# maple3142/gf2bv

Hardware: AMD Instinct MI355X
Metric: GF(2) row-XORs/s (solve_one, dense NxN) (higher is better)
Workload: dtype u64

## Files before the change

### gf2bv_amd/csrc/gf2_kernels.hip.h

```cpp
#pragma once
#include <hip/hip_runtime.h>
#include <stdint.h>
#include <type_traits>

typedef unsigned long long u64;
typedef long long i64;

#define GF2_GMAX 4
#define GF2_TW 2
#define GF2_TW_LOG 1
#define GF2_LPR 1
#define GF2_OWN_LOG 3
#define GF2_FEW_UNITS 8
#ifndef GF2_BATCH
#define GF2_BATCH 4
#endif
#ifndef GF2_UROWS
#define GF2_UROWS 2
#endif

__device__ __forceinline__ long long tidx(long long row, long long word, long long srows)
{
	return ((word >> GF2_TW_LOG) * srows + row) * GF2_TW + (word & (GF2_TW - 1));
}
// ... 2536 lines not shown
			u32x4 v[NB][RB];
			loadm(0, 0); loadm(1, 1);
#pragma unroll
			for (int pre = 0; pre < NB - 1; pre++) issue(v[pre], m0[0], m1[0], pre);
#pragma unroll
			for (int j = 0; j < SEG; j++) {
#pragma unroll
				for (int rr = 0; rr < NR; rr++) {
					const int g = j * NR + rr;
					const int gi = g + NB - 1, ji = gi / NR, ri = gi % NR, ci = ji & 1;
					issue(v[gi % NB], m0[ci], m1[ci], ri);
					if (ri == NR - 1) loadm(ji + 2, ci);
					fold(d[j], v[g % NB]);
				}
			}
		}
#pragma unroll
		for (int j = 0; j < SEG; j++)
			if ((alive >> j) & 1) (Mrow + j * (NW * 64))[ulane] = d[j];
	}
}

#define GF2_U16K_PARAMS u64 *__restrict__ M, i64 rows, i64 srows, int nblk, const int *__restrict__ gprow, const u64 *__restrict__ mult, i64 set_words, \
	int set0, int nsets, const int *__restrict__ blk_first, const int *__restrict__ died, int j_end, int tile_begin, int ntiles, SysStride ss, int chunk_major
#define GF2_U16K_ARGS M, rows, srows, nblk, gprow, mult, set_words, set0, nsets, blk_first, died, j_end, tile_begin, ntiles, ss, chunk_major
template <int SEG, int NT_ = 512, int RB = 8, int NB = 2>
__global__ void __launch_bounds__(NT_)
k_update16k(GF2_U16K_PARAMS)
{
	update16k_body<SEG, NT_, RB, NB>(GF2_U16K_ARGS);
}
#define GF2_WSEG 12
#define GF2_U16K_WIDE(NAME, SEG, RB, NB, VB) \
	__global__ void __launch_bounds__(1024) __attribute__((amdgpu_num_vgpr(VB))) NAME(GF2_U16K_PARAMS) { update16k_body<SEG, 1024, RB, NB>(GF2_U16K_ARGS); }
GF2_U16K_WIDE(k_update16k_wide, GF2_WSEG, 2, 2, 60)

__global__ void __launch_bounds__(512)
k_outer_apply(u64 *__restrict__ M, i64 rows, i64 srows, int nblk, const int *__restrict__ lists, const u64 *__restrict__ Tm, int tile_begin, SysStride ss)
{
	{
		const i64 ao = blockIdx.y * ss.arena_bytes;
		M += blockIdx.y * ss.m_words;
		lists = sys_at(lists, ao); Tm = sys_at(Tm, ao);
	}
	constexpr int NT = 512, NW = 8, SEG = GF2_KMAX * GF2_GMAX * 64 / NT, NQ = GF2_KMAX * GF2_GMAX * 64;
	__shared__ __attribute__((aligned(256))) uint4 tab[2 * 256 * 16];
	__shared__ uint4 stage[GF2_GMAX * 64];
	__shared__ int srcrow[NQ];
	if ((unsigned)(size_t)tab != 0u) __builtin_trap();
	const int lane = threadIdx.x & 63, wv = threadIdx.x >> 6;
	const int wvu = __builtin_amdgcn_readfirstlane(wv);
	for (int t = threadIdx.x; t < NQ; t += NT) srcrow[t] = lists[NQ + GF2_KMAX + t];
	__syncthreads();
	unsigned KC[6];
	{
		const int rq_lo = lane & 7, rq_hi = (lane >> 3) & 1;
#pragma unroll
		for (int v = 0; v < 6; v++) {
			unsigned k = 1u << 24;
#pragma unroll
			for (int b = 0; b < 3; b++) {
				const int s = 3 * v + b;
				if (s < 16) k |= (unsigned)(16 * (8 * ((s >> 3) ^ rq_hi) + (((s & 7) + rq_lo) & 7))) << (8 * b);
			}
			asm volatile("" : "+v"(k));
			KC[v] = k;
		}
	}
	const i64 R64 = (rows + 63) & ~(i64)63;
	uint4 *Mw = reinterpret_cast<uint4 *>(M) + ((i64)tile_begin + blockIdx.x) * srows;
	uint4 d[SEG];
#pragma unroll
	for (int j = 0; j < SEG; j++) d[j] = make_uint4(0, 0, 0, 0);
	uint4 staged = make_uint4(0, 0, 0, 0);
	if (threadIdx.x < GF2_GMAX * 64) { const int sr = srcrow[threadIdx.x]; staged = sr >= 0 ? Mw[sr] : make_uint4(0, 0, 0, 0); }
	const uint4 *tbase = reinterpret_cast<const uint4 *>(Tm);
#pragma unroll 1
	for (int k = 0; k < nblk; k++) {
		const uint4 *mq = tbase + (i64)k * (NQ * 2);
		uint4 A0[SEG], A1[SEG];
#pragma unroll
		for (int j = 0; j < SEG; j++) {
			const int i = (j * NW + wv) * 64 + lane;
			if (((j * NW + wvu) >> 2) < k) { A0[j] = make_uint4(0, 0, 0, 0); A1[j] = A0[j]; }
			else { A0[j] = mq[i * 2]; A1[j] = mq[i * 2 + 1]; }
		}
		__syncthreads();
		if (threadIdx.x < GF2_GMAX * 64) stage[threadIdx.x] = staged;
		__syncthreads();
		for (int e = threadIdx.x; e < 2 * 31 * 16; e += NT) {
			const int sub = e & 15, q = (e >> 4) % 31, grp = (e >> 4) / 31;
			const int idx = q <= 15 ? q : (q - 15) << 4;
			const uint4 *st = stage + (2 * grp + (sub >> 3)) * 64 + 8 * (sub & 7);
			uint4 acc = make_uint4(0, 0, 0, 0);
			int bits = idx;
			while (bits) { const int l = __ffs(bits) - 1; bits &= bits - 1; acc = xor4(acc, st[l]); }
			tab[grp * 4096 + idx * 16 + sub] = acc;
		}
		__syncthreads();
		for (int e = threadIdx.x; e < 2 * 225 * 16; e += NT) {
			const int sub = e & 15, q = (e >> 4) % 225, grp = (e >> 4) / 225;
			const int lo = 1 + q % 15, hi = (1 + q / 15) << 4;
			uint4 *tb = tab + grp * 4096 + sub;
			tb[(lo | hi) * 16] = xor4(tb[lo * 16], tb[hi * 16]);
		}
		if (k + 1 < nblk && threadIdx.x < GF2_GMAX * 64) {
			const int sr = srcrow[(k + 1) * 256 + threadIdx.x];
			staged = sr >= 0 ? Mw[sr] : make_uint4(0, 0, 0, 0);
		}
		__syncthreads();
#pragma unroll
		for (int j = 0; j < SEG; j++) {
			if (((j * NW + wvu) >> 2) < k) continue;
			const uint4 a0 = A0[j], a1 = A1[j];
			const unsigned mw[8] = { a0.x, a0.y, a0.z, a0.w, a1.x, a1.y, a1.z, a1.w };
#pragma unroll
			for (int r = 0; r < 4; r++) {
				const int grp = r >> 1, hf = r & 1;
				u32x4 v[8];
#pragma unroll
				for (int q = 0; q < 8; q++) {
					const int s = 8 * hf + q;
					const unsigned sel = (unsigned)(s % 3) | ((4u + (unsigned)(q & 3)) << 8) | ((grp ? 3u : 12u) << 16) | (12u << 24);
					const unsigned at = __builtin_amdgcn_perm(mw[2 * (2 * grp + hf) + (q >> 2)], KC[s / 3], sel);
					v[q] = *(lds_u4_ptr)(size_t)at;
				}
#pragma unroll
				for (int h = 0; h < 4; h++) {
					d[j].x = __builtin_amdgcn_bitop3_b32(d[j].x, v[2 * h].x, v[2 * h + 1].x, 0x96);
					d[j].y = __builtin_amdgcn_bitop3_b32(d[j].y, v[2 * h].y, v[2 * h + 1].y, 0x96);
					d[j].z = __builtin_amdgcn_bitop3_b32(d[j].z, v[2 * h].z, v[2 * h + 1].z, 0x96);
					d[j].w = __builtin_amdgcn_bitop3_b32(d[j].w, v[2 * h].w, v[2 * h + 1].w, 0x96);
				}
			}
		}
	}
#pragma unroll
	for (int j = 0; j < SEG; j++) {
		const int i = (j * NW + wv) * 64 + lane;
		const int pr = srcrow[i];
		Mw[pr >= 0 ? (i64)pr : R64] = d[j];
	}
}



__global__ void __launch_bounds__(256)
k_check_rhs(const u64 *__restrict__ M, i64 rows, i64 srows, i64 cols,
            const int *__restrict__ died, SolveState *__restrict__ st, SysStride ss)
{
	M += blockIdx.y * ss.m_words;
	died = sys_at(died, blockIdx.y * ss.arena_bytes);
	st = sys_at(st, blockIdx.y * ss.arena_bytes);
	int bad = 0;
	for (i64 i = (i64)blockIdx.x * blockDim.x + threadIdx.x; i < rows; i += (i64)gridDim.x * blockDim.x)
		if (died[i] == GF2_NEVER) bad |= (int)((M[tidx(i, cols >> 6, srows)] >> (cols & 63)) & 1);
	if (__ballot(bad) && (threadIdx.x & 63) == 0) st->inconsistent = 1;
}


__device__ __forceinline__ u64 wave_or64(u64 v)
{
#pragma unroll
	for (int m = 32; m >= 1; m >>= 1) {
		const unsigned lo = (unsigned)__shfl_xor((int)(unsigned)v, m), hi = (unsigned)__shfl_xor((int)(unsigned)(v >> 32), m);
		v |= ((u64)hi << 32) | lo;
	}
	return v;
}

__global__ void __launch_bounds__(256)
k_check_rhs_many(const u64 *__restrict__ M, i64 rows, i64 srows, i64 cols, i64 nrhs, const int *__restrict__ died,
                 u64 *__restrict__ bad)
{
	const int s = (int)(cols & 63);
	const i64 nrw = (s + nrhs + 63) / 64, nmw = (nrhs + 63) / 64;
	for (i64 k = blockIdx.y; k < nrw; k += gridDim.y) {
		const i64 q = (cols >> 6) + k;
		u64 acc = 0;
		for (i64 i = (i64)blockIdx.x * blockDim.x + threadIdx.x; i < rows; i += (i64)gridDim.x * blockDim.x)
			if (died[i] == GF2_NEVER) acc |= M[tidx(i, q, srows)];
		acc = wave_or64(acc);
		if ((threadIdx.x & 63) == 0) {
			if (k < nmw && (acc >> s)) atomicOr(&bad[k], acc >> s);
			if (s && k >= 1 && (acc << (64 - s))) atomicOr(&bad[k - 1], acc << (64 - s));
		}
	}
}

__device__ __forceinline__ u64 rhs_block_transposed(const u64 *__restrict__ rhs, i64 nrhs, i64 rhs_words, i64 m, i64 rb, int lane)
{
	if (m < 0 || m * 64 >= nrhs) return 0;
	const i64 j = m * 64 + lane;
	const u64 x = j < nrhs ? rhs[j * rhs_words + rb] : 0ull;
	u64 mine = 0;
	for (int i = 0; i < 64; i++) {
		const u64 b = __ballot((x >> i) & 1);
		if (lane == i) mine = b;
	}
	return mine;
}

__global__ void __launch_bounds__(256)
k_pack_rhs(const u64 *__restrict__ rhs, i64 nrhs, i64 rhs_words, i64 rows, i64 cols, i64 srows, u64 *__restrict__ M)
{
	const int lane = threadIdx.x & 63;
	const i64 rb = (i64)blockIdx.x * 4 + (threadIdx.x >> 6);
	if (rb * 64 >= rows) return;
	const int s = (int)(cols & 63);
	const i64 nrw = (s + nrhs + 63) / 64, r = rb * 64 + lane;
	for (i64 k = blockIdx.y; k < nrw; k += gridDim.y) {
		const u64 cur = rhs_block_transposed(rhs, nrhs, rhs_words, k, rb, lane);
		u64 v = cur << s;
		if (s) v |= rhs_block_transposed(rhs, nrhs, rhs_words, k - 1, rb, lane) >> (64 - s);
		if (r < rows) {
			u64 &w = M[tidx(r, (cols >> 6) + k, srows)];
			if (k == 0) v |= w & ((1ull << s) - 1);
			w = v;
		}
	}
}


__global__ void __launch_bounds__(256)
k_factor_init(i64 rows, i64 cols, i64 srows, i64 tw0, i64 rw, u64 *__restrict__ M)
{
	const i64 r = (i64)blockIdx.x * blockDim.x + threadIdx.x;
	if (r >= rows) return;
	const int s = (int)(cols & 63);
	const i64 q0 = cols >> 6, q1 = tw0 + rw, mine = tw0 + (r >> 6);
	for (i64 q = q0 + blockIdx.y; q < q1; q += gridDim.y) {
		u64 &w = M[tidx(r, q, srows)];
		if (q == q0) w &= (1ull << s) - 1;
		else w = q == mine ? 1ull << (r & 63) : 0ull;
	}
}

#define GF2_FT_WORDS 64
__global__ void __launch_bounds__(256)
k_apply_transform(const u64 *__restrict__ M, i64 rows, i64 srows, i64 tw0, i64 rw, const u64 *__restrict__ rhs, int nrhs,
                  i64 rhs_stride, u64 *__restrict__ acc)
{
	__shared__ ulonglong2 sb[GF2_FT_WORDS / 2][64];
	const i64 w0 = (i64)blockIdx.y * GF2_FT_WORDS, wn = rw - w0 < GF2_FT_WORDS ? rw - w0 : GF2_FT_WORDS;
	for (int i = threadIdx.x; i < (GF2_FT_WORDS / 2) * nrhs; i += blockDim.x) {
		const int j = i / (GF2_FT_WORDS / 2), p = i % (GF2_FT_WORDS / 2);
		const u64 *b = rhs + (i64)j * rhs_stride + w0;
		sb[p][j] = make_ulonglong2(2 * p < wn ? b[2 * p] : 0ull, 2 * p + 1 < wn ? b[2 * p + 1] : 0ull);
	}
	__syncthreads();
	const i64 r = (i64)blockIdx.x * blockDim.x + threadIdx.x;
	if (r >= rows) return;
	u64 out = 0;
	for (int p = 0; 2 * p < wn; p++) {
		const ulonglong2 t = *reinterpret_cast<const ulonglong2 *>(&M[tidx(r, tw0 + w0 + 2 * p, srows)]);
		for (int j = 0; j < nrhs; j++) {
			const ulonglong2 b = sb[p][j];
			out ^= (u64)(__popcll((t.x & b.x) ^ (t.y & b.y)) & 1) << j;
		}
	}
	if (out) atomicXor(&acc[r], out);
}

__global__ void __launch_bounds__(256)
k_put_rhs(const u64 *__restrict__ acc, i64 rows, i64 cols, i64 srows, u64 *__restrict__ M)
{
	const i64 r = (i64)blockIdx.x * blockDim.x + threadIdx.x;
	if (r >= rows) return;
	const int s = (int)(cols & 63);
	const u64 a = acc[r], low = (1ull << s) - 1;
	u64 &w0 = M[tidx(r, cols >> 6, srows)];
	w0 = (w0 & low) | (a << s);
	if (s) {
		u64 &w1 = M[tidx(r, (cols >> 6) + 1, srows)];
		w1 = (w1 & ~low) | (a >> (64 - s));
	}
}


__global__ void __launch_bounds__(256)
k_append_retile(const u64 *__restrict__ src, i64 srows_old, i64 rows_old, i64 ntiles_old, u64 *__restrict__ dst, i64 srows_new,
                i64 ntiles_new)
{
	const i64 r = (i64)blockIdx.x * blockDim.x + threadIdx.x;
	if (r >= srows_new) return;
	for (i64 t = blockIdx.y; t < ntiles_new; t += gridDim.y) {
		ulonglong2 v = make_ulonglong2(0ull, 0ull);
		if (t < ntiles_old && r < rows_old) v = reinterpret_cast<const ulonglong2 *>(src)[t * srows_old + r];
		reinterpret_cast<ulonglong2 *>(dst)[t * srows_new + r] = v;
	}
}

__global__ void __launch_bounds__(256)
k_append_init(i64 r0, i64 k, i64 cols, i64 srows, i64 tw0, i64 wend, u64 *__restrict__ M)
{
	const i64 i = (i64)blockIdx.x * blockDim.x + threadIdx.x;
	if (i >= k) return;
	const i64 r = r0 + i;
	const int s = (int)(cols & 63);
	const i64 q0 = cols >> 6, mine = tw0 + (r >> 6);
	for (i64 q = q0 + blockIdx.y; q < wend; q += gridDim.y) {
		u64 &w = M[tidx(r, q, srows)];
		if (q == q0) w &= (1ull << s) - 1;
		else w = q == mine ? 1ull << (r & 63) : 0ull;
	}
}
// ... 31 lines not shown
#pragma unroll
		for (int u = 0; u < 8; u++)
			v[u] = reinterpret_cast<const ulonglong2 *>(M)[t * srows + srow[j0 + u < rec.p ? j0 + u : j0]];
#pragma unroll
		for (int u = 0; u < 8; u++) {
			if (j0 + u >= rec.p) break;
			const int b = sbit[j0 + u];
			if (!((y >> b) & 1)) continue;
			const u64 above = ~rec.mask & (~0ull << b << 1);
			a0 ^= wt0 < w ? 0ull : (wt0 == w ? v[u].x & above : v[u].x);
			a1 ^= wt0 + 1 == w ? v[u].y & above : v[u].y;
		}
	}
	if (!on) return;
	ulonglong2 &d = reinterpret_cast<ulonglong2 *>(M)[t * srows + r0 + i];
	ulonglong2 o = d;
	o.x ^= a0; o.y ^= a1;
	if (wt0 == w) o.x &= ~rec.mask;
	if (wt0 + 1 == w) o.y &= ~rec.mask;
	d = o;
	if (wnext == wt0) snap_next[i] = o.x;
	if (wnext == wt0 + 1) snap_next[i] = o.y;
}

__global__ void __launch_bounds__(256)
k_append_gather(const u64 *__restrict__ M, i64 srows, i64 r0, i64 k, const int *__restrict__ fc, i64 nf, i64 nfw, i64 ldw,
                u64 *__restrict__ W)
{
	const i64 e = (i64)blockIdx.x * blockDim.x + threadIdx.x;
	if (e >= k * ldw) return;
	const i64 i = e / ldw, q = e % ldw;
	u64 v = 0;
	if (q < nfw) {
		const i64 j0 = q * 64, n = nf - j0 < 64 ? nf - j0 : 64;
		for (i64 b = 0; b < n; b++) {
			const int c = fc[j0 + b];
			v |= ((M[tidx(r0 + i, c >> 6, srows)] >> (c & 63)) & 1) << b;
		}
	} else if (q - nfw == (i >> 6)) v = 1ull << (i & 63);
	W[e] = v;
}

__global__ void __launch_bounds__(1024)
k_append_eliminate(u64 *__restrict__ W, int k, i64 nfw, i64 ldw, int *__restrict__ out_col, int *__restrict__ out_row,
                   int *__restrict__ out_n)
{
	__shared__ unsigned long long best;
	__shared__ u64 has[16];
	const int t = threadIdx.x;
	bool alive = t < k;
	i64 lq = 0;
	int n = 0;
	for (;;) {
		if (t == 0) best = ~0ull;
		if (t < 16) has[t] = 0;
		__syncthreads();
		if (alive) {
			const u64 *row = W + (i64)t * ldw;
			while (lq < nfw && row[lq] == 0) lq++;
			if (lq < nfw) {
				const u64 lead = (u64)(lq * 64 + __ffsll((long long)row[lq]) - 1);
				atomicMin(&best, (lead << 10) | (u64)t);
			}
		}
		__syncthreads();
		const u64 bk = best;
		if (bk == ~0ull) break;
		const int p = (int)(bk & 1023);
		const i64 c = (i64)(bk >> 10), cq = c >> 6;
		if (t < k && t != p && ((W[(i64)t * ldw + cq] >> (c & 63)) & 1)) atomicOr(&has[t >> 6], 1ull << (t & 63));
		if (t == p) alive = false;
		if (t == 0) { out_col[n] = (int)c; out_row[n] = p; }
		n++;
		__syncthreads();
		const i64 span = ldw - cq;
		const u64 *prow = W + (i64)p * ldw + cq;
		for (i64 e = t; e < (i64)k * span; e += blockDim.x) {
			const i64 i = e / span, q = e % span;
			if ((has[i >> 6] >> (i & 63)) & 1) W[i * ldw + cq + q] ^= prow[q];
		}
		__syncthreads();
	}
	if (t == 0) *out_n = n;
}

__global__ void __launch_bounds__(256)
k_append_combine(u64 *__restrict__ M, i64 srows, i64 r0, int k, i64 ntiles, const u64 *__restrict__ W, i64 nfw, i64 ldw)
{
	__shared__ ulonglong2 B[1024];
	for (i64 t = blockIdx.x; t < ntiles; t += gridDim.x) {
		ulonglong2 *tile = reinterpret_cast<ulonglong2 *>(M) + t * srows + r0;
		for (int i = threadIdx.x; i < k; i += blockDim.x) B[i] = tile[i];
		__syncthreads();
		for (int i = threadIdx.x; i < k; i += blockDim.x) {
			const u64 *e = W + (i64)i * ldw + nfw;
			ulonglong2 o = make_ulonglong2(0ull, 0ull);
			for (int q = 0; q * 64 < k; q++) {
				u64 m = e[q];
				while (m) {
					const int j = q * 64 + __ffsll((long long)m) - 1;
					m &= m - 1;
					o.x ^= B[j].x; o.y ^= B[j].y;
				}
			}
			tile[i] = o;
		}
		__syncthreads();
	}
}

__global__ void __launch_bounds__(256)
k_append_backreduce(u64 *__restrict__ M, i64 srows, i64 ntiles, const int4 *__restrict__ items, const int *__restrict__ nbit,
                    const int *__restrict__ nrow)
{
	const int4 it = items[blockIdx.x];
	const int row = it.x, w = it.y, b = it.z >> 8, n = it.z & 255, first = it.w;
	__shared__ u64 ssel;
	if (threadIdx.x == 0) {
		const u64 own = M[tidx(row, w, srows)];
		u64 sel = 0;
		for (int j = 0; j < n; j++) {
			const int nb = nbit[first + j];
			if (nb > b && ((own >> nb) & 1)) sel |= 1ull << j;
		}
		ssel = sel;
	}
	__syncthreads();
	const u64 sel = ssel;
	if (!sel) return;
	for (i64 t = (w >> 1) + threadIdx.x; t < ntiles; t += blockDim.x) {
		ulonglong2 &d = reinterpret_cast<ulonglong2 *>(M)[t * srows + row];
		ulonglong2 o = d;
		for (u64 m = sel; m; m &= m - 1) {
			const int j = __ffsll((long long)m) - 1;
			const ulonglong2 v = reinterpret_cast<const ulonglong2 *>(M)[t * srows + nrow[first + j]];
			if (t * 2 >= w) o.x ^= v.x;
			o.y ^= v.y;
		}
		d = o;
	}
}

__global__ void __launch_bounds__(256)
k_append_died(int *__restrict__ died, const int *__restrict__ row, const int *__restrict__ val, int n)
{
	const int j = blockIdx.x * blockDim.x + threadIdx.x;
	if (j < n) died[row[j]] = val[j];
}

#define GF2_BSG 16
#define GF2_BSV 8
#define GF2_BS_MAXRHS 64

__global__ void __launch_bounds__(256)
k_bs_far(const u64 *__restrict__ M, i64 srows, i64 cw, int qa, int qb, const PanelRec *__restrict__ panels,
         const int *__restrict__ urow, const int *__restrict__ pivcol, const int *__restrict__ ycols, int ny,
         const u64 *__restrict__ X, unsigned char *__restrict__ accv, i64 nacc, SysStride ss, i64 x_sys_words)
{
	{
		const i64 ao = blockIdx.y * ss.arena_bytes;
		M += blockIdx.y * ss.m_words; X += blockIdx.y * x_sys_words;
		panels = sys_at(panels, ao); urow = sys_at(urow, ao); pivcol = sys_at(pivcol, ao); accv = sys_at(accv, ao);
	}
	const int lane = threadIdx.x & 63;
	const i64 wv = ((i64)blockIdx.x * blockDim.x + threadIdx.x) >> 6;
	const int kbeg = panels[qa].start;
	const int kend = panels[qb - 1].start + panels[qb - 1].p;
	const i64 k = kbeg + wv;
	if (k >= kend) return;
	const i64 row = urow[k];
	u64 par[GF2_BSV];
#pragma unroll
	for (int v = 0; v < GF2_BSV; v++) par[v] = 0;
	for (i64 w = qb + lane; w < cw; w += 64) {
		const u64 m = M[tidx(row, w, srows)];
#pragma unroll
		for (int v = 0; v < GF2_BSV; v++)
			if (v < ny) par[v] ^= m & X[(i64)v * cw + w];
	}
	const int pw = pivcol[k] >> 6;
#pragma unroll
	for (int v = 0; v < GF2_BSV; v++) {
		if (v >= ny) break;
		int bit = __popcll(par[v]) & 1;
		bit = __popcll(__ballot(bit)) & 1;
		const int c = ycols[v];
		const int y = ((c >> 6) >= pw) ? (int)((M[tidx(row, c >> 6, srows)] >> (c & 63)) & 1) : 0;
		if (lane == 0) accv[(i64)v * nacc + k] = (unsigned char)(bit ^ y);
	}
}

#define GF2_BSINV_LDS (16 * 64 * 16 * 8 + 256 * 8 * 8 + 1024 + 64)
__global__ void __launch_bounds__(1024)
k_bs_inv(const u64 *__restrict__ Dg, int npanels, const PanelRec *__restrict__ panels, const int *__restrict__ pivcol,
         u64 *__restrict__ Minv)
{
	extern __shared__ __attribute__((aligned(16))) u64 lds_inv[];
	u64 *R = lds_inv;
	u64 *T = R + 16 * 64 * 16;
	unsigned char *pcs = reinterpret_cast<unsigned char *>(T + 256 * 8);
	const int g = blockIdx.x, qb = npanels - g * GF2_BSG, qa = qb > GF2_BSG ? qb - GF2_BSG : 0, nb = qb - qa;
	const int t = threadIdx.x;
	{
		const int i = t >> 6, r = t & 63;
		unsigned char pc = 255;
		if (i < nb) { const PanelRec rec = panels[qa + i]; if (r < rec.p) pc = (unsigned char)(pivcol[rec.start + r] & 63); }
		pcs[t] = pc;
	}
	for (int e = t; e < 16 * 64 * 16; e += 1024) R[e] = 0;
	__syncthreads();
	if (pcs[t] != 255) { const int i = t >> 6; R[(i * 64 + pcs[t]) * 16 + i] = 1ull << pcs[t]; }
	__syncthreads();
	for (int j = nb - 1; j >= 1; j--) {
		const int nrows = j * 64;
		for (int h = (j >> 3); h < 2; h++) {
			for (int e = t; e < 256 * 8; e += 1024) {
				const int nv = e >> 3, w = e & 7, n = nv >> 4, v = nv & 15;
				u64 a0 = R[(j * 64 + 4 * n + 0) * 16 + 8 * h + w], a1 = R[(j * 64 + 4 * n + 1) * 16 + 8 * h + w];
				u64 a2 = R[(j * 64 + 4 * n + 2) * 16 + 8 * h + w], a3 = R[(j * 64 + 4 * n + 3) * 16 + 8 * h + w];
				if (!(v & 1)) a0 = 0;
				if (!(v & 2)) a1 = 0;
				if (!(v & 4)) a2 = 0;
				if (!(v & 8)) a3 = 0;
				T[e] = (a0 ^ a1) ^ (a2 ^ a3);
			}
			__syncthreads();
			const int w0 = (j > 8 * h) ? j - 8 * h : 0, nw = 8 - w0;
			for (int e = t; e < nrows * nw; e += 1024) {
				const int row = e % nrows, w = w0 + e / nrows;
				const unsigned char pc = pcs[row];
				if (pc == 255) continue;
				const int i = row >> 6, r = row & 63;
				const u64 u = Dg[((i64)(qa + i) * 64 + r) * 16 + (j - i - 1)];
				if (!u) continue;
				u64 v16[16];
#pragma unroll
				for (int n = 0; n < 16; n++) v16[n] = T[(n * 16 + (int)((unsigned)(u >> (4 * n)) & 15u)) * 8 + w];
				u64 acc = 0;
#pragma unroll
				for (int n = 0; n < 16; n += 2) acc ^= v16[n] ^ v16[n + 1];
				R[(i * 64 + pc) * 16 + 8 * h + w] ^= acc;
			}
			__syncthreads();
		}
	}
	u64 *dst = Minv + (i64)g * (16 * 64 * 16);
	for (int e = t; e < 16 * 64 * 16; e += 1024) dst[e] = R[e];
}

__global__ void __launch_bounds__(1024)
k_bs_near2(i64 cw, int qa, int qb, const PanelRec *__restrict__ panels, const int *__restrict__ pivcol, int ny,
           u64 *__restrict__ X, const unsigned char *__restrict__ accv, i64 nacc, const u64 *__restrict__ Minv, int gidx)
{
	__shared__ u64 aL[GF2_BSG];
	const int lane = threadIdx.x & 63, i = threadIdx.x >> 6, nb = qb - qa;
	const bool onp = i < nb;
	const uint4 *rowp = reinterpret_cast<const uint4 *>(Minv + (i64)gidx * (16 * 64 * 16) + ((i64)(onp ? i : 0) * 64 + lane) * 16);
	uint4 q[8];
#pragma unroll
	for (int z = 0; z < 8; z++) q[z] = rowp[z];
	const PanelRec rec = panels[qa + (onp ? i : 0)];
	const int kk = rec.start + lane;
	const bool piv = onp && lane < rec.p;
	const int pcb = piv ? (pivcol[kk] & 63) : 0;
	for (int v = 0; v < ny; v++) {
		const u64 word = wave_or(piv ? (u64)(accv[(i64)v * nacc + kk] & 1) << pcb : 0ull);
		if (lane == 0) aL[i] = word;
		__syncthreads();
		u64 acc = 0;
#pragma unroll
		for (int z = 0; z < 8; z++)
			acc ^= ((((u64)q[z].y << 32) | q[z].x) & aL[2 * z]) ^ ((((u64)q[z].w << 32) | q[z].z) & aL[2 * z + 1]);
		const u64 xw = __ballot(__popcll(acc) & 1);
		if (lane == 0 && onp) X[(i64)v * cw + qa + i] = xw;
		__syncthreads();
	}
}

__global__ void __launch_bounds__(256)
k_bs_diag(const u64 *__restrict__ M, i64 srows, int npanels, const PanelRec *__restrict__ panels,
          const int *__restrict__ urow, u64 *__restrict__ Dg, SysStride ss, i64 dg_sys_words)
{
	{
		const i64 ao = blockIdx.y * ss.arena_bytes;
		M += blockIdx.y * ss.m_words; Dg += blockIdx.y * dg_sys_words;
		panels = sys_at(panels, ao); urow = sys_at(urow, ao);
	}
	const int q = blockIdx.x, t = threadIdx.x;
	const int r = t >> 2, q4 = t & 3;
	const PanelRec rec = panels[q];
	const bool on = r < rec.p;
	const int ur0 = urow[on ? rec.start + r : 0];
	const int ur = on ? ur0 : 0;
	u64 v[4];
#pragma unroll
	for (int m = 0; m < 4; m++) {
		const int w = q + 1 + 4 * q4 + m;
		v[m] = M[tidx(ur, w < npanels ? w : q, srows)];
		if (!on || w >= npanels) v[m] = 0;
	}
	uint4 *dst = reinterpret_cast<uint4 *>(Dg + ((i64)q * 64 + r) * 16 + 4 * q4);
	dst[0] = make_uint4((unsigned)v[0], (unsigned)(v[0] >> 32), (unsigned)v[1], (unsigned)(v[1] >> 32));
	dst[1] = make_uint4((unsigned)v[2], (unsigned)(v[2] >> 32), (unsigned)v[3], (unsigned)(v[3] >> 32));
}

__global__ void __launch_bounds__(256)
k_bs_near(const u64 *__restrict__ Dg, i64 cw, int qa, int qb, const PanelRec *__restrict__ panels,
          const int *__restrict__ pivcol, int ny, u64 *__restrict__ X,
          const unsigned char *__restrict__ accv, i64 nacc, SysStride ss, i64 dg_sys_words, i64 x_sys_words)
{
	{
		const i64 ao = blockIdx.y * ss.arena_bytes;
		Dg += blockIdx.y * dg_sys_words; X += blockIdx.y * x_sys_words;
		panels = sys_at(panels, ao); pivcol = sys_at(pivcol, ao); accv = sys_at(accv, ao);
	}
	__shared__ u64 Xn[GF2_BSG + 4];
	const int t = threadIdx.x;
	const int r = t >> 2, q4 = t & 3;
	const int nb = qb - qa;
	u64 uw[GF2_BSG][4];
	int kk[GF2_BSG], pc[GF2_BSG];
	PanelRec rec[GF2_BSG];
#pragma unroll
	for (int i = 0; i < GF2_BSG; i++) rec[i] = panels[qa + (i < nb ? i : 0)];
#pragma unroll
	for (int i = 0; i < GF2_BSG; i++) {
		const uint4 *src = reinterpret_cast<const uint4 *>(Dg + ((i64)(qa + (i < nb ? i : 0)) * 64 + r) * 16 + 4 * q4);
		const uint4 a = src[0], b = src[1];
		const bool on = i < nb && r < rec[i].p;
		const int k = on ? rec[i].start + r : 0;
		kk[i] = on ? k : -1;
		pc[i] = pivcol[k] & 63;
		const u64 x[4] = { ((u64)a.y << 32) | a.x, ((u64)a.w << 32) | a.z, ((u64)b.y << 32) | b.x, ((u64)b.w << 32) | b.z };
#pragma unroll
		for (int m = 0; m < 4; m++) uw[i][m] = (on && qa + i + 1 + 4 * q4 + m < qb) ? x[m] : 0ull;
	}
	for (int v = 0; v < ny; v++) {
		if (t < GF2_BSG + 4) Xn[t] = 0;
		unsigned ac = 0;
#pragma unroll
		for (int i = 0; i < GF2_BSG; i++)
			if (kk[i] >= 0) ac |= (unsigned)(accv[(i64)v * nacc + kk[i]] & 1) << i;
		__syncthreads();
#pragma unroll
		for (int i = GF2_BSG - 1; i >= 0; i--) {
			if (i >= nb) continue;
			int par = 0;
#pragma unroll
			for (int m = 0; m < 4; m++) {
				const int xi = i + 1 + 4 * q4 + m;
				if (xi < GF2_BSG + 4) par ^= __popcll(uw[i][m] & Xn[xi]);
			}
			par ^= __builtin_amdgcn_update_dpp(0, par, 0xb1, 0xf, 0xf, false);
			par ^= __builtin_amdgcn_update_dpp(0, par, 0x4e, 0xf, 0xf, false);
			const bool set = q4 == 0 && kk[i] >= 0 && ((par ^ (int)(ac >> i)) & 1);
			const u64 bits = wave_or(set ? 1ull << pc[i] : 0ull);
			if ((t & 63) == 0 && bits) atomicOr(&Xn[i], bits);
			__syncthreads();
		}
		if (t < nb) X[(i64)v * cw + qa + t] = Xn[t];
		__syncthreads();
	}
}

__global__ void __launch_bounds__(256)
k_extract_y(const u64 *__restrict__ M, i64 srows, const SolveState *__restrict__ st,
            const int *__restrict__ urow, const int *__restrict__ pivcol,
            const int *__restrict__ ycols, int ny, u64 *__restrict__ Y, i64 ys, i64 k0)
{
	const int lane = threadIdx.x & 63;
	const i64 wave = ((i64)blockIdx.x * blockDim.x + threadIdx.x) >> 6;
	const int nyw = (ny + 63) >> 6;
	const i64 k = k0 + wave / nyw;
	const int tw = (int)(wave % nyw);
	if (k >= st->rank) return;
	const int t = tw * 64 + lane;
	int bit = 0;
	if (t < ny) {
		const int c = ycols[t];
		if ((c >> 6) >= (pivcol[k] >> 6))
			bit = (int)((M[tidx(urow[k], c >> 6, srows)] >> (c & 63)) & 1);
	}
	const u64 w = __ballot(bit);
	if (lane == 0) Y[k * ys + tw] = w;
}

__global__ void __launch_bounds__(256)
k_gather_mult_u(const u64 *__restrict__ M, i64 srows, int j, const PanelRec *__restrict__ rec,
                const int *__restrict__ urow, u64 *__restrict__ mult)
{
	const int p = rec->p;
	if (p == 0) return;
	const i64 hi = rec->start;
	const u64 mask = rec->mask;
	for (i64 k = (i64)blockIdx.x * blockDim.x + threadIdx.x; k < hi; k += (i64)gridDim.x * blockDim.x)
		mult[k] = M[tidx(urow[k], j, srows)] & mask;
}

template <int K, int TW>
struct SweepCfg {
	static constexpr int T = (64 + K - 1) / K;
	static constexpr int LASTBITS = 64 - K * (T - 1);
	static constexpr int ENTRIES = (T - 1) * (1 << K) + (1 << LASTBITS);
	static constexpr int LPR = TW / 2;
	static constexpr int LDS_BYTES = ENTRIES * TW * 8;
};

template <int K, int TW, int NT>
__global__ void __launch_bounds__(NT)
k_sweep(u64 *__restrict__ M, i64 stride, i64 rows_total, const PanelRec *__restrict__ rec,
        int above, const u64 *__restrict__ mult, int tile0, int ntiles, int rows_per_block)
{
	typedef SweepCfg<K, TW> C;
	extern __shared__ __attribute__((aligned(16))) uint4 tab[];
	const int p = rec->p;
	if (p == 0) return;
	const int start = rec->start;
	const u64 pmask = rec->mask;
	const i64 lo = above ? 0 : (i64)start + p;
	const i64 hi = above ? (i64)start : rows_total;
	const int ct = blockIdx.x % ntiles;
	const i64 rb = blockIdx.x / ntiles;
	const i64 rbeg = lo + rb * rows_per_block;
	if (rbeg >= hi) return;
	const i64 rend = (rbeg + rows_per_block < hi) ? rbeg + rows_per_block : hi;
	const i64 w0 = (i64)(tile0 + ct) * TW;
	const int lr = threadIdx.x % C::LPR;
	const int rr = threadIdx.x / C::LPR;
	constexpr int RPP = NT / C::LPR;

	const uint4 *Mq = reinterpret_cast<const uint4 *>(M);
	for (int g = rr; g < C::ENTRIES; g += RPP) {
		int t = g >> K; if (t > C::T - 1) t = C::T - 1;
		const int idx = g - (t << K);
		const int kt = (t == C::T - 1) ? C::LASTBITS : K;
		const int kl = kt >> 1;
		const int lomask = (1 << kl) - 1;
		if ((idx & lomask) && (idx & ~lomask)) continue;
		uint4 acc = make_uint4(0, 0, 0, 0);
		int bits = idx;
		while (bits) {
			int l = __ffs(bits) - 1; bits &= bits - 1;
			int b = t * K + l;
			if ((pmask >> b) & 1) {
				i64 prow = (i64)start + __popcll(pmask & ((1ull << b) - 1));
				acc = xor4(acc, Mq[(prow * stride + w0) / 2 + lr]);
			}
		}
		tab[g * C::LPR + lr] = acc;
	}
	__syncthreads();
	for (int g = rr; g < C::ENTRIES; g += RPP) {
		int t = g >> K; if (t > C::T - 1) t = C::T - 1;
		const int idx = g - (t << K);
		const int kt = (t == C::T - 1) ? C::LASTBITS : K;
		const int kl = kt >> 1;
		const int lomask = (1 << kl) - 1;
		if (!((idx & lomask) && (idx & ~lomask))) continue;
		const int base = g - idx;
		tab[g * C::LPR + lr] = xor4(tab[(base + (idx & lomask)) * C::LPR + lr], tab[(base + (idx & ~lomask)) * C::LPR + lr]);
	}
	__syncthreads();

	uint4 *Mw = reinterpret_cast<uint4 *>(M);
	constexpr int U = 4;
	for (i64 base = rbeg; base < rend; base += (i64)RPP * U) {
		u64 m[U];
		uint4 d[U];
		i64 q[U];
#pragma unroll
		for (int u = 0; u < U; u++) {
			i64 row = base + (i64)u * RPP + rr;
			m[u] = (row < rend) ? mult[row] : 0ull;
			q[u] = (row * stride + w0) / 2 + lr;
		}
#pragma unroll
		for (int u = 0; u < U; u++)
			if (m[u]) d[u] = Mw[q[u]];
#pragma unroll
		for (int u = 0; u < U; u++) {
			if (!m[u]) continue;
			uint4 acc = d[u];
#pragma unroll
			for (int t = 0; t < C::T; t++) {
				const int kt = (t == C::T - 1) ? C::LASTBITS : K;
				const unsigned idx = (unsigned)(m[u] >> (K * t)) & ((1u << kt) - 1);
				acc = xor4(acc, tab[((t << K) + idx) * C::LPR + lr]);
			}
			Mw[q[u]] = acc;
		}
	}
}

__global__ void __launch_bounds__(256)
k_scatter_solution(const u64 *__restrict__ Y, i64 ys, const SolveState *__restrict__ st,
                   const int *__restrict__ pivcol, int ny, u64 *__restrict__ out, i64 cw, i64 k0)
{
	const int nyw = (ny + 63) >> 6;
	const i64 g = (i64)blockIdx.x * blockDim.x + threadIdx.x;
	const i64 k = k0 + g / nyw;
	const int tw = (int)(g % nyw);
	if (k >= st->rank) return;
	u64 y = Y[k * ys + tw];
	const int c = pivcol[k];
	while (y) {
		int b = ctz64(y); y &= y - 1;
		i64 t = (i64)tw * 64 + b;
		if (t < ny) atomicOr(&out[t * cw + (c >> 6)], 1ull << (c & 63));
	}
}

__global__ void __launch_bounds__(256)
k_space_enumerate(const u64 *__restrict__ origin, const u64 *__restrict__ basis, int dim, i64 words, u64 first,
                  i64 count, int gray, u64 *__restrict__ out)
// ... 1633 lines not shown
```

### gf2bv_amd/csrc/gf2_solver.hip

```cpp
#include "gf2_kernels.hip.h"
#include <hip/hip_ext.h>
#include "../../include/gf2bv_hip.h"

#include <algorithm>
#include <array>
#include <atomic>
#include <chrono>
#include <cstdio>
#include <cstdlib>
#include <cstring>
#include <functional>
#include <map>
#include <memory>
#include <new>
#include <mutex>
#include <string>
#include <thread>
#include <unordered_map>
#include <vector>

namespace {

thread_local std::string g_err = "";

// ... 370 lines not shown
			if (!c) {
				int lo = 0, hi = 0;
				(void)hipDeviceGetStreamPriorityRange(&lo, &hi);
				if ((err = hipStreamCreateWithPriority(&c, hipStreamNonBlocking, lo)) != hipSuccess) break;
			}
			int all_ok = 1;
			for (hipStream_t x : with) {
				int ok = -1;
				{
					std::lock_guard<std::mutex> lk(mu);
					auto it = pair_ok.find({x, c});
					if (it != pair_ok.end()) ok = it->second;
				}
				if (ok < 0) {
					ok = 1;
					if (probe_pair(x, c, device, &ok, kn) != hipSuccess) { (void)hipGetLastError(); ok = 1; }
					else {
						std::lock_guard<std::mutex> lk(mu);
						pair_ok[{x, c}] = ok;
						pairs_probed++; pairs_bad += !ok;
					}
				}
				if (!ok) { all_ok = 0; break; }
			}
			if (all_ok) *out = c; else rejected.push_back(c);
		}
		if (!*out && !rejected.empty()) { *out = rejected.front(); rejected.erase(rejected.begin()); }
		for (hipStream_t r : rejected) release_stream(r, device, cls);
		if (!*out && err == hipSuccess) return stream(out, device, cls);
		return err;
	}
};
Pool &pool()
{
	static Pool *p = new Pool();
	return *p;
}
int alloc_or_nomem(void **out, size_t bytes, int device, const char *nomem, const char *what)
{
	const hipError_t e = pool().alloc(out, bytes, device);
	if (e == hipErrorOutOfMemory) { (void)hipGetLastError(); return fail(GF2BV_ERR_NOMEM, nomem); }
	if (e != hipSuccess) return fail(GF2BV_ERR_HIP, what, e);
	return GF2BV_OK;
}

int streams_run_concurrently(const Knobs &kn, int device, hipStream_t a, hipStream_t b, int *ok);
int xcd_dispatch_is_round_robin(int device, hipStream_t st, int *ok);
void forget_concurrency(int device);

struct UpdateImpl {
	int G, T, lds_bytes, threads;
	hipError_t (*update)(dim3, hipStream_t, u64 *, i64, i64, int, int, int, const PanelRec *, const PanelAux *,
	                     const u64 *, const int *, int, int, int, int, int, bool, const uint4 *, SysStride, hipEvent_t, hipEvent_t, int);
};

template <int NT, int DEPTH, bool PIPE, int LB>
hipError_t launch_update16(dim3 grid, hipStream_t s, u64 *M, i64 rows, i64 srows, int j0, int gb, int wlo,
                           const PanelRec *panels, const PanelAux *aux, const u64 *multset, const int *blk_first,
                           int tile_begin, int ntiles, int world, int wrank, int nw_lo, bool stream_rows, const uint4 *Pc, SysStride ss,
                           hipEvent_t begun, hipEvent_t done, int xcd_nsys)
{
	if (xcd_nsys > 0) grid = dim3(grid.x * grid.y);
	{
		if (stream_rows && NT == 512 && DEPTH == 3 && PIPE && LB == 512) {
			if (nw_lo < 0)
				hipExtLaunchKernelGGL((k_update16<512, true, 3, true, 512, true>), grid, dim3(512), 0, s, begun, done, 0, M, rows, srows, j0, gb, wlo,
				                      panels, aux, multset, blk_first, tile_begin, ntiles, world, wrank, Pc, ss, xcd_nsys);
			else
				hipExtLaunchKernelGGL((k_update16<512, false, 3, true, 512, true>), grid, dim3(512), 0, s, begun, done, 0, M, rows, srows, j0, gb, wlo,
				                      panels, aux, multset, blk_first, tile_begin, ntiles, world, wrank, Pc, ss, xcd_nsys);
			return hipGetLastError();
		}
	}
	if (nw_lo < 0)
		hipExtLaunchKernelGGL((k_update16<NT, true, DEPTH, PIPE, LB>), grid, dim3(NT), 0, s, begun, done, 0, M, rows, srows, j0, gb, wlo,
		                      panels, aux, multset, blk_first, tile_begin, ntiles, world, wrank, Pc, ss, xcd_nsys);
	else
		hipExtLaunchKernelGGL((k_update16<NT, false, DEPTH, PIPE, LB>), grid, dim3(NT), 0, s, begun, done, 0, M, rows, srows, j0, gb, wlo,
		                      panels, aux, multset, blk_first, tile_begin, ntiles, world, wrank, Pc, ss, xcd_nsys);
	return hipGetLastError();
}
#define UPDATE16_IMPL(NT, D, P, LB) { 4, 8, 2 * 256 * 256 + GF2_GMAX * 64 * 20, NT, launch_update16<NT, D, P, LB> }

const UpdateImpl kUpdates[] = {
	UPDATE16_IMPL(512, 3, true, 512),
	UPDATE16_IMPL(768, 2, true, 768),
	UPDATE16_IMPL(768, 2, true, 1024),
	UPDATE16_IMPL(1024, 2, false, 1024),
	UPDATE16_IMPL(768, 3, true, 768),
	UPDATE16_IMPL(640, 2, true, 640),
};

static_assert(sizeof kUpdates / sizeof kUpdates[0] == Knobs::kNumUpdates, "GF2BV_UPDATE indexes this table");

constexpr int YK = 5, YTW = 16, YNT = 1024;
hipError_t launch_ysweep(dim3 grid, hipStream_t s, u64 *Y, i64 ys, i64 rows, const PanelRec *rec,
                         const u64 *mult, int ntiles, int rpb)
{
	constexpr int lds = SweepCfg<YK, YTW>::LDS_BYTES;
	static std::mutex attr_mu;
	static std::map<int, bool> attr_set;
	int dev = 0;
	(void)hipGetDevice(&dev);
	{
		std::lock_guard<std::mutex> lk(attr_mu);
		if (!attr_set[dev]) {
			hipError_t e = hipFuncSetAttribute((const void *)k_sweep<YK, YTW, YNT>,
			                                   hipFuncAttributeMaxDynamicSharedMemorySize, lds);
			if (e != hipSuccess) return e;
			attr_set[dev] = true;
		}
	}
	k_sweep<YK, YTW, YNT><<<grid, dim3(YNT), lds, s>>>(Y, ys, rows, rec, 1, mult, 0, ntiles, rpb);
	return hipGetLastError();
}

constexpr int TW = GF2_TW;

inline size_t round256(size_t bytes) { return (bytes + 255) & ~(size_t)255; }

struct ArenaLayout {
	size_t st = 0, sf = 0, panels = 0, aux = 0, fu = 0, died = 0, pivcol = 0, urow = 0, blk_first = 0, mult = 0, Wb = 0, Uwin = 0, Pfast = 0,
	       oprow = 0, Tm = 0, Pc = 0, wmask = 0, stride = 0;
};

struct SolverPlan {
	int device = 0;
	i64 rows = 0, cols = 0, stride = 0;
	i64 ntiles = 0, srows = 0;
	int nsys = 1;
	int gang_nsys = 1;
	int world = 1, wrank = 0;
	i64 m_stride = 0, src_sys_words = 0;
	ArenaLayout lay;
	bool view = false;
	bool own_bs = true;
	SysStride ss() const { return SysStride{ m_stride, (i64)lay.stride }; }
	int mode = 0;
	int nrhs = 1;
	bool time_kernels = false;
	Knobs kn;
	const UpdateImpl *impl = nullptr;

	int nsets = 2;
	int tl_K = 0, tl_bend = 0;
	i64 tile_hi = 0;
	static constexpr int nlist = 2;
	bool bulk_waits_outer = false;
	bool ends_outer_panel(int b) const { return tl_K > 0 && b < tl_bend && (b + 1) % tl_K == 0; }
	bool flag_sync = true;
	bool optimistic = true;
	bool xcd_pin = true;
	int sync_base = 0;
	int units = 0;
	bool sparse_on = false;
	int sparse_giveups = 0;
	int sparse_tier = 0;
	int narrow_rpt = 1;
	i64 ys = 0;
	int ny = 0;
	int h_ycol = 0;
	i64 maxr = 0;
	int npanels = 0, nblocks = 0;
	i64 wt = 0, cw = 0;

	std::vector<int> free_order;
	SolveState hst{};
	std::vector<u64> hout;
	std::vector<PanelRec> hp;
	std::vector<int32_t> hpiv;
	std::chrono::steady_clock::time_point t_begin;
	float ms_pack = 0;
};

ArenaLayout arena_layout(const SolverPlan &P)
{
	const i64 R = std::max<i64>(1, P.rows), NP = std::max(1, P.npanels);
	const int G = P.impl->G;
	ArenaLayout L;
	size_t off = 0;
	auto carve = [&](size_t bytes) { size_t at = off; off += round256(bytes); return at; };
	L.st = carve(sizeof(SolveState)); L.sf = carve(sizeof(SyncFlags)); L.panels = carve(sizeof(PanelRec) * NP); L.aux = carve(sizeof(PanelAux) * NP);
	L.fu = carve(sizeof(FindUnit) * (P.units + 1 + GF2_MAXGROUPS)); L.died = carve(sizeof(int) * (size_t)R);
	L.pivcol = carve(sizeof(int) * (P.maxr + 64)); L.urow = carve(sizeof(int) * (P.maxr + 64));
	L.blk_first = carve(sizeof(int) * std::max(1, P.nblocks)); L.mult = carve(sizeof(u64) * P.nsets * G * mult_rows(R) + (P.tl_K ? kOuterSlackBytes : 0));
	L.Wb = carve(sizeof(u64) * 2 * GF2_GMAX * R); L.Uwin = carve(sizeof(u64) * GF2_GMAX * (P.maxr + 64));
	L.Pfast = carve(sizeof(u64) * GF2_GMAX * GF2_GMAX * 64); L.oprow = carve(sizeof(int) * GF2_OUTER_LISTS * P.nlist);
	L.Tm = carve(P.tl_K ? P.nlist * sizeof(u64) * GF2_KMAX * GF2_KMAX * GF2_GMAX * 64 * GF2_GMAX : 0);
	L.Pc = carve(P.kn.pc ? sizeof(u64) * 2 * GF2_GMAX * 64 * (size_t)P.ntiles : 0);
	L.wmask = carve(sizeof(u64) * 2 * (size_t)((R + 63) / 64 + 1));
	L.stride = off;
	return L;
}

struct ArenaPtrs {
	SolveState *st = nullptr;
	SyncFlags *sf = nullptr;
	PanelRec *panels = nullptr;
	PanelAux *aux = nullptr;
	FindUnit *fu = nullptr;
	int *died = nullptr;
	int *pivcol = nullptr, *urow = nullptr, *blk_first = nullptr;
	u64 *mult = nullptr;
	u64 *Wb = nullptr;
	u64 *Uwin = nullptr;
	u64 *Pfast = nullptr;
	int *oprow = nullptr;
	u64 *Tm = nullptr;
	u64 *Pc = nullptr;
	u64 *wmask = nullptr;

	void bind(const ArenaLayout &L, void *arena, bool pc)
	{
		char *base = (char *)arena;
		st = (SolveState *)(base + L.st); sf = (SyncFlags *)(base + L.sf); panels = (PanelRec *)(base + L.panels); aux = (PanelAux *)(base + L.aux);
		fu = (FindUnit *)(base + L.fu); died = (int *)(base + L.died); pivcol = (int *)(base + L.pivcol); urow = (int *)(base + L.urow);
		blk_first = (int *)(base + L.blk_first); mult = (u64 *)(base + L.mult); Wb = (u64 *)(base + L.Wb); Uwin = (u64 *)(base + L.Uwin);
		Pfast = (u64 *)(base + L.Pfast); oprow = (int *)(base + L.oprow); Tm = (u64 *)(base + L.Tm);
		Pc = pc ? (u64 *)(base + L.Pc) : nullptr;
		wmask = (u64 *)(base + L.wmask);
	}
};

struct SolverHandles {
	hipStream_t sA = nullptr, sB = nullptr;
	bool own_sA = false, own_sB = false;
	u64 *M = nullptr;
	bool ext_M = false;
	const u64 *src = nullptr;
	u64 *tmp_src = nullptr;
	u64 *Minv = nullptr;
	u64 *rhs_bad = nullptr;
	void *arena = nullptr;
	hipStream_t sC = nullptr;
	hipEvent_t evOuter = nullptr, evPri = nullptr, evPanelDone = nullptr, evBig = nullptr;
	u64 *Y = nullptr;
	int *ycols = nullptr;
	u64 *out = nullptr;
	hipEvent_t ev0 = nullptr, ev1 = nullptr, ev2 = nullptr, ev3 = nullptr;
	std::vector<hipEvent_t> evA, evPrio, kev, waitPrio;
	hipEvent_t evx = nullptr;
};

struct Solver : SolverPlan, ArenaPtrs, SolverHandles {
	SolverPlan &plan() { return *this; }
	const SolverPlan &plan() const { return *this; }
	Solver() = default;
	Solver(const Solver &) = delete;
	Solver &operator=(const Solver &) = delete;
	~Solver() { release(); }
	void release()
	{
		if (!arena && !M && !tmp_src && !Y && !ycols && !out && !sA && !sB && !ev0) return;
		(void)hipSetDevice(device);
		Pool &P = pool();
		if (view) {
			if (sA && (Y || ycols || out)) (void)hipStreamSynchronize(sA);
			if (own_bs) for (void *p : { (void *)Y, (void *)ycols, (void *)out, (void *)Minv }) P.release(p);
			P.release_event(ev2, true);
			P.release_event(evx, true);
			arena = nullptr; M = nullptr; sA = sB = nullptr; ev0 = ev1 = ev3 = nullptr;
		} else {
			if (sC) (void)hipStreamSynchronize(sC);
			if (sB) (void)hipStreamSynchronize(sB);
			if (arena || M) (void)hipStreamSynchronize(sA);
			for (void *p : { arena, (void *)Y, (void *)ycols, (void *)out, (void *)Minv, (void *)(ext_M ? nullptr : M), (void *)tmp_src }) P.release(p);
			for (hipEvent_t e : { ev0, ev1, ev2, ev3, evx }) P.release_event(e, true);
			for (hipEvent_t e : { evOuter, evPri, evPanelDone, evBig }) P.release_event(e, false);
			if (sC) P.release_stream(sC, device, nsys > 1 ? 3 : 1);
			for (hipEvent_t e : kev) P.release_event(e, true);
			for (hipEvent_t e : evA) P.release_event(e, false);
			for (hipEvent_t e : evPrio) P.release_event(e, false);
			if (own_sB && sB) P.release_stream(sB, device, nsys > 1 ? 3 : 1);
			if (own_sA && sA) P.release_stream(sA, device, false);
		}
		static_cast<ArenaPtrs &>(*this) = ArenaPtrs();
		static_cast<SolverHandles &>(*this) = SolverHandles();
	}
};

}

struct gf2bv_result {
	int status = 0;
	i64 rank = 0, dim = 0, cw = 0;
	std::vector<u64> origin, basis;
	std::vector<int32_t> pivots;
	gf2bv_stats stats{};
};

namespace {

struct Scratch {
	std::vector<void *> bufs;
	std::vector<hipEvent_t> timing_events;
	hipStream_t sync_first = nullptr;
	~Scratch()
	{
		if (sync_first) (void)hipStreamSynchronize(sync_first);
		for (void *p : bufs) pool().release(p);
		for (hipEvent_t e : timing_events) pool().release_event(e, true);
	}
	hipError_t alloc(void **out, size_t bytes, int device)
	{
		hipError_t e = pool().alloc(out, bytes, device);
		if (e == hipSuccess) bufs.push_back(*out);
		return e;
	}
	hipError_t event(hipEvent_t *ev)
	{
		hipError_t e = pool().event(ev, true);
		if (e == hipSuccess) timing_events.push_back(*ev);
		return e;
	}
};

int check_device(int device)
{
	int n = 0;
	hipError_t e = hipGetDeviceCount(&n);
	if (e != hipSuccess || n <= 0)
		return fail(GF2BV_ERR_NODEVICE, "no HIP device visible: gf2bv_amd has no CPU fallback");
	if (device < 0 || device >= n) return fail(GF2BV_ERR_ARG, "device index out of range");
	HIPCHK(hipSetDevice(device));
	return GF2BV_OK;
}

void plan_two_level(Solver &S)
{
	S.tl_K = 0; S.tl_bend = 0; S.nsets = 2;
	if (S.world != 1 || S.ext_M || S.impl->G != GF2_GMAX) return;
	if (S.nsys != 1) return;
	int K = (double)S.rows * (double)S.wt * 8.0 >= 3.0 * 1073741824.0 ? GF2_KMAX : 8;
	double min_bytes = 0.5 * 1073741824.0;
	if (S.kn.two_level == 0) return;
	if (S.kn.two_level > 0) { K = S.kn.two_level; min_bytes = 0; }
	if (S.kn.two_level_min_set) min_bytes = 1048576.0 * S.kn.two_level_min_mib;
	const int G = S.impl->G;
	int bend = 0;
	for (int b0 = 0; b0 + K < S.nblocks; b0 += K) {
		const i64 rows_left = S.rows - (i64)(b0 + K) * 64 * G, words_left = S.wt - (i64)(b0 + K) * G;
		if ((i64)(b0 + K) * 64 * G > S.cols || rows_left <= 0 || words_left <= 0) break;
		if ((double)rows_left * (double)words_left * 8.0 * (double)S.nsys < min_bytes) break;
		bend = b0 + K;
	}
	if (!bend) return;
	S.tl_K = K; S.tl_bend = bend;
	S.nsets = 2 * K;
}

int solver_alloc(Solver &S)
{
	const Knobs &kn = S.kn = Knobs::read();
	S.wt = (S.cols + S.nrhs + 63) / 64;
	S.cw = (S.cols + 63) / 64;
	S.npanels = (int)((S.cols + 63) / 64);
	S.maxr = std::min(S.rows, S.cols);
	S.impl = &kUpdates[S.kn.update];
	S.ntiles = tiles_for(S.wt);
	S.srows = slab_rows(S.rows);
	S.m_stride = S.ntiles * TW * S.srows;
	if (!S.M) HIPCHK(pool().alloc((void **)&S.M, sizeof(u64) * S.m_stride * S.nsys + kOuterSlackBytes, S.device));
	if (S.src && S.rows > 0) {
		k_to_tiled<<<dim3((unsigned)((S.rows + 63) / 64), (unsigned)((S.ntiles + 15) / 16), S.nsys), dim3(256), 0, S.sA>>>(
			S.src, S.stride, S.rows, S.ntiles, std::min(S.wt, S.stride), S.srows, S.M, S.src_sys_words, S.ss());
	}
	const int G = S.impl->G;
	S.nblocks = (S.npanels + G - 1) / G;
	S.tile_hi = S.ntiles;
	plan_two_level(S);
	S.units = (int)std::min<i64>(256, std::max<i64>(1, (S.rows + 255) / 256));
	S.flag_sync = S.world == 1 && !kn.plain && kn.flag_sync != 0 && !kn.serial;
	S.optimistic = kn.optimistic >= 0 ? kn.optimistic != 0 : !kn.plain;
	S.xcd_pin = kn.xcd_pin >= 0 ? kn.xcd_pin != 0 : !kn.plain;
	if (kn.xcd_pin < 0 && !kn.plain && S.nsys >= 8 && S.nsys % 8 == 0) {
		int ok = 0;
		int rc = xcd_dispatch_is_round_robin(S.device, S.sA, &ok);
		if (rc) return rc;
		S.xcd_pin = ok != 0;
	}
	{
		const i64 blocks = (S.rows + 255) / 256 * std::max(1, S.nsys);
		S.narrow_rpt = (int)std::min<i64>(8, std::max<i64>(1, blocks / 256));
	}
	if (kn.serial) { S.sB = S.sA; S.own_sB = false; }
	else {
		if (S.nsys == 1) HIPCHK(pool().low_stream_for(kn, S.sA, S.device, &S.sB));
		else HIPCHK(pool().stream(&S.sB, S.device, 3));
		S.own_sB = true;
	}
	if (S.flag_sync && S.sB != S.sA) {
		int ok = 0;
		int rc = streams_run_concurrently(kn, S.device, S.sA, S.sB, &ok);
		if (rc) return rc;
		S.flag_sync = ok != 0;
	}
	{
		const ArenaLayout &L = S.lay = arena_layout(S);
		S.sync_base = 0;
		HIPCHK(pool().alloc(&S.arena, L.stride * S.nsys, S.device));
		S.bind(L, S.arena, kn.pc);
		for (int s = 0; s < S.nsys; s++) {
			char *b = (char *)S.arena + (size_t)s * L.stride;
			HIPCHK(hipMemsetAsync(b + L.st, 0, L.died - L.st, S.sA));
			HIPCHK(hipMemsetAsync(b + L.died, GF2_NEVER & 0xff, sizeof(int) * (size_t)std::max<i64>(1, S.rows), S.sA));
			HIPCHK(hipMemsetAsync(b + L.blk_first, 0, L.Wb - L.blk_first, S.sA));
		}
	}
	HIPCHK(pool().event(&S.ev0, true));
	HIPCHK(pool().event(&S.ev1, true));
	HIPCHK(pool().event(&S.ev2, true));
	HIPCHK(pool().event(&S.ev3, true));
	if (S.tl_K) {
		for (hipEvent_t *e : { &S.evOuter, &S.evPri, &S.evPanelDone }) HIPCHK(pool().event(e, false));
		if (S.sB != S.sA) { if (S.nsys == 1) HIPCHK(pool().low_stream_for(kn, S.sA, S.device, &S.sC)); else HIPCHK(pool().stream(&S.sC, S.device, 3)); }
		HIPCHK(pool().event(&S.evBig, false));
	}
	S.evA.resize(S.nblocks); S.evPrio.resize(S.nblocks); S.waitPrio.assign(S.nblocks, nullptr);
	for (int b = 0; b < S.nblocks; b++) {
// ... 193 lines not shown
		k_win_scatter<<<dim3((unsigned)((S.rows * g.gb + 255) / 256), S.nsys), dim3(256), 0, S.sA>>>(S.M, S.rows, S.srows, g.j0, g.gb, half[g.gb & 1], S.died, S.st, S.ss());
	HIPCHK(hipGetLastError());
	if (S.flag_sync) { int rc = panel_handover(S, b); if (rc) return rc; }
	else if (b == S.nblocks - 1) HIPCHK(hipEventRecord(S.evA[b], S.sA));
	if (S.kn.debug_sync & 1) HIPCHK(hipDeviceSynchronize());
	return GF2BV_OK;
}

int enqueue_block_bulk(Solver &S, int b)
{
	const BlockGeom g = block_geom(S, b);
	if (S.bulk_waits_outer) { HIPCHK(hipStreamWaitEvent(S.sB, S.evOuter, 0)); S.bulk_waits_outer = false; }
	if (S.flag_sync) {
		k_gate<<<dim3(1, S.nsys), dim3(64), 0, S.sB>>>(S.sf, S.st, 0, S.sync_base + b, S.sync_base + b + 1, 0, S.ss());
		HIPCHK(hipGetLastError());
	} else HIPCHK(hipStreamWaitEvent(S.sB, S.evA[b], 0));
	bool launched = false;
	if (g.nt_all > 0) {
		int rc = launch_trsm(S, S.sB, g.j0, g.gb, g.wlo, g.wlo, g.wlo + g.gnext);
		if (rc) return rc;
		const int wend = g.wlo + g.gnext;
		const int tfull = g.gnext > 0 ? (wend + 1) / 2 : g.wlo / 2;
		const i64 nfull = owned_count(tfull, S.tile_hi, GF2_OWN_LOG - 1, S.world, S.wrank);
		if ((wend & 1) && g.gnext > 0 && owned_count(wend / 2, wend / 2 + 1, GF2_OWN_LOG - 1, S.world, S.wrank) > 0) {
			rc = launch_update_timed(S, S.sB, b, g.j0, g.gb, g.wlo, g.mset, wend / 2, 1, -1, nfull <= 0, &S.waitPrio[b]);
			if (rc) return rc;
			launched = nfull <= 0;
		}
		if (nfull > 0) {
			rc = launch_update_timed(S, S.sB, b, g.j0, g.gb, g.wlo, g.mset, tfull, (int)nfull, 0, true, &S.waitPrio[b]);
			if (rc) return rc;
			launched = true;
		}
	}
	if (!launched && !S.flag_sync) {
		HIPCHK(hipEventRecord(S.evPrio[b], S.sB));
		S.waitPrio[b] = S.evPrio[b];
	}
	if (S.kn.debug_sync & 2) HIPCHK(hipDeviceSynchronize());
	return GF2BV_OK;
}

int enqueue_block_prio(Solver &S, int b)
{
	if (b + 1 >= S.nblocks || S.ends_outer_panel(b)) return GF2BV_OK;
	const BlockGeom g = block_geom(S, b);
	const unsigned row_blocks = (unsigned)((S.rows + 255) / 256);
	if (b > 0 && !S.flag_sync) HIPCHK(hipStreamWaitEvent(S.sA, S.waitPrio[b - 1], 0));
	if (b > 0 && S.flag_sync) {
		k_gate<<<dim3(1, S.nsys), dim3(64), 0, S.sA>>>(S.sf, S.st, 0, 0, 0, S.sync_base + b, S.ss());
		HIPCHK(hipGetLastError());
	}
	k_prio_window<<<dim3(row_blocks, S.nsys), dim3(256), 0, S.sA>>>(S.M, S.rows, S.srows, g.j0, g.gb, g.wlo, std::max(g.gnext, 1),
	                                                             S.panels, S.aux, g.mset, S.blk_first + b, S.Wb, S.Uwin,
	                                                             S.impl->T, S.st, S.ss(), (const int *)S.died, S.sparse_on ? S.wmask : (u64 *)nullptr);
	HIPCHK(hipGetLastError());
	return GF2BV_OK;
}

int enqueue_forward_begin(Solver &S, bool gather_first_window)
{
	HIPCHK(hipEventRecord(S.ev0, S.sA));
	HIPCHK(hipStreamWaitEvent(S.sB, S.ev0, 0));
	if (S.npanels > 0 && gather_first_window) {
		const int g0 = std::min(S.impl->G, S.npanels);
		k_win_gather<<<dim3((unsigned)((S.rows * g0 + 255) / 256), S.nsys), dim3(256), 0, S.sA>>>(S.M, S.rows, S.srows, 0, g0, S.Wb, S.st, S.ss());
	}
	return GF2BV_OK;
}

int enqueue_forward_join(Solver &S)
{
	HIPCHK(hipEventRecord(S.ev3, S.sB));
	HIPCHK(hipStreamWaitEvent(S.sA, S.ev3, 0));
	if (S.nblocks > 1 && S.maxr > 0)
		k_unwind<<<dim3((unsigned)((S.maxr * GF2_GMAX + 255) / 256), S.nsys), dim3(256), 0, S.sA>>>(
			S.M, S.srows, S.impl->G, S.npanels, S.nblocks, S.st, S.pivcol, S.urow, S.Uwin, S.world, S.wrank, S.tl_K, S.tl_bend, S.ss());
	HIPCHK(hipGetLastError());
	return GF2BV_OK;
}

int enqueue_check_rhs(Solver &S)
{
	int g = (int)std::min<i64>(1024, (S.rows + 255) / 256);
	if (S.rhs_bad) {
		const i64 nrw = ((S.cols & 63) + S.nrhs + 63) / 64;
		k_check_rhs_many<<<dim3(g, (unsigned)std::min<i64>(nrw, 65535)), dim3(256), 0, S.sA>>>(S.M, S.rows, S.srows, S.cols, S.nrhs,
		                                                                                      S.died, S.rhs_bad);
	} else {
		k_check_rhs<<<dim3(g, S.nsys), dim3(256), 0, S.sA>>>(S.M, S.rows, S.srows, S.cols, S.died, S.st, S.ss());
	}
	HIPCHK(hipGetLastError());
	HIPCHK(hipEventRecord(S.ev1, S.sA));
	return GF2BV_OK;
}

int enqueue_outer_prepare(Solver &S, hipStream_t st, int b0, int b1)
{
	const int G = S.impl->G;
	const i64 set_words = (i64)G * mult_rows(S.rows);
	const int npan = (b1 - b0) * G;
	int *gprow = S.oprow + (size_t)((b0 / S.tl_K) % S.nlist) * GF2_OUTER_LISTS;
	u64 *Tm = S.Tm + (size_t)((b0 / S.tl_K) % S.nlist) * ((size_t)GF2_KMAX * GF2_KMAX * GF2_GMAX * 64 * GF2_GMAX);
	k_outer_prow<<<dim3(1, S.nsys), dim3(256), 0, st>>>(b0 * G, b1 - b0, S.panels, S.aux, gprow, S.ss());
	if (!S.kn.outer_chain)
		k_outer_trsm<4, true><<<dim3((unsigned)(npan / 4), S.nsys), dim3(256), 0, st>>>(S.M, S.rows, S.srows, b0 * G, npan, 0, S.panels, S.aux, S.mult,
		                                                                               set_words, b0 % S.nsets, S.nsets, S.impl->T, Tm, S.ss());
	HIPCHK(hipGetLastError());
	return GF2BV_OK;
}

int enqueue_outer_apply(Solver &S, hipStream_t st, int b0, int b1, i64 t_begin, i64 t_end)
{
	const int G = S.impl->G;
	const i64 nt = t_end - t_begin;
	if (nt <= 0) return GF2BV_OK;
	const i64 set_words = (i64)G * mult_rows(S.rows);
	int *gprow = S.oprow + (size_t)((b0 / S.tl_K) % S.nlist) * GF2_OUTER_LISTS;
	const int npan = (b1 - b0) * G;
	if (S.kn.outer_chain) {
		const i64 g_begin = t_begin * TW / 4, ng = t_end * TW / 4 - g_begin;
		k_outer_trsm<4, false><<<dim3((unsigned)ng, S.nsys), dim3(256), 0, st>>>(S.M, S.rows, S.srows, b0 * G, npan, (int)g_begin, S.panels, S.aux,
		                                                                          S.mult, set_words, b0 % S.nsets, S.nsets, S.impl->T, (u64 *)nullptr, S.ss());
	} else
		k_outer_apply<<<dim3((unsigned)nt, S.nsys), dim3(512), 0, st>>>(S.M, S.rows, S.srows, b1 - b0, (const int *)gprow,
		                                                                (const u64 *)(S.Tm + (size_t)((b0 / S.tl_K) % S.nlist) * ((size_t)GF2_KMAX * GF2_KMAX * GF2_GMAX * 64 * GF2_GMAX)), (int)t_begin, S.ss());
	HIPCHK(hipGetLastError());
	hipEvent_t ka = nullptr, kb = nullptr;
	if (S.time_kernels) {
		HIPCHK(pool().event(&ka, true)); HIPCHK(pool().event(&kb, true));
		S.kev.push_back(ka); S.kev.push_back(kb);
	}
	const i64 est_lo = std::min<i64>(S.rows, (i64)b0 * 64 * G) & ~(i64)63, R64 = round_up(S.rows, 64);
	constexpr i64 item_rows = (i64)GF2_WSEG * 1024;
	static_assert((size_t)item_rows * 32 <= kOuterSlackBytes, "the slack behind the matrix covers an item");
	const i64 nch = std::max<i64>(1, (R64 - est_lo + item_rows - 1) / item_rows);
	const i64 wgs = std::min<i64>(nch * nt, (i64)1 << 30);
	hipExtLaunchKernelGGL(k_update16k_wide, dim3((unsigned)wgs, S.nsys), dim3(1024), 0, st, ka, kb, 0,
	                      S.M, S.rows, S.srows, b1 - b0, (const int *)gprow, (const u64 *)S.mult,
	                      set_words, b0 % S.nsets, S.nsets, (const int *)(S.blk_first + b0), (const int *)S.died, b1 * G, (int)t_begin, (int)nt, S.ss(), 1);
	HIPCHK(hipGetLastError());
	if (S.kn.debug_sync & 2) HIPCHK(hipDeviceSynchronize());
	return GF2BV_OK;
}

int enqueue_window_gather(Solver &S, int b)
{
	const BlockGeom g = block_geom(S, b);
	k_win_gather<<<dim3((unsigned)((S.rows * g.gb + 255) / 256), S.nsys), dim3(256), 0, S.sA>>>(S.M, S.rows, S.srows, g.j0, g.gb, S.Wb, S.st, S.ss());
	HIPCHK(hipGetLastError());
	return GF2BV_OK;
}

int enqueue_forward(Solver &S)
{
	Trace tr;
	int rc = enqueue_forward_begin(S, true);
	if (rc) return rc;
	bool optimistic = false;
	SolveState hst{};
	const bool may_probe = S.kn.fast && S.optimistic && S.nsys == 1 && S.world == 1 && S.nblocks >= 8 && fast_block_possible(S, block_geom(S, 0));
	auto fast_only_ok = [&](int blk) {
		return fast_block_possible(S, block_geom(S, blk)) && S.rows - (i64)blk * 64 * S.impl->G >= GF2_FAST_NC + 128;
	};
	const bool may_sparse = may_probe && S.kn.sparse_fast && S.tl_K == 0;
	int general_only = -1;
	auto sparse_ok = [&](int blk) { return S.sparse_on && blk != general_only && fast_block_possible(S, block_geom(S, blk)); };
	auto recover = [&](int pb) -> int {
		if (S.sC) HIPCHK(hipStreamSynchronize(S.sC));
		HIPCHK(hipStreamSynchronize(S.sB));
		if (S.tl_K && pb < S.tl_bend) S.tl_bend = pb / S.tl_K * S.tl_K;
		S.bulk_waits_outer = false;
		HIPCHK(hipMemsetAsync(&S.st->poison, 0, sizeof(int), S.sA));
		S.sync_base += S.nblocks + 1;
		return GF2BV_OK;
	};
	int sparse_probes = 1;
	auto one_block = [&](int blk) -> int {
		int r;
		bool sp = sparse_ok(blk);
		if ((r = enqueue_block_panel(S, blk, sp || (optimistic && fast_only_ok(blk)), sp))) return r;
		if (sp && sparse_probes > 0) {
			sparse_probes--;
			HIPCHK(hipMemcpyAsync(&hst, S.st, sizeof hst, hipMemcpyDeviceToHost, S.sA));
			HIPCHK(hipStreamSynchronize(S.sA));
			const int want = hst.sp_nz > 3400 ? 2 : 0;
			if (hst.poison) {
				if ((r = recover(blk))) return r;
				if (++S.sparse_giveups >= 3) S.sparse_on = false; else sparse_probes = 1;
				S.sparse_tier = std::min(2, std::max(S.sparse_tier + 1, want));
				general_only = blk;
				if ((r = enqueue_block_panel(S, blk, false, false))) return r;
			} else S.sparse_tier = std::max(S.sparse_tier, want);
		}
		if ((r = enqueue_block_bulk(S, blk))) return r;
		if ((r = enqueue_block_prio(S, blk))) return r;
		if (blk == 0 && may_probe) {
			HIPCHK(hipMemcpyAsync(&hst, S.st, sizeof hst, hipMemcpyDeviceToHost, S.sA));
			HIPCHK(hipStreamSynchronize(S.sA));
			optimistic = hst.fast_done == 1;
			if (!optimistic && may_sparse && S.nblocks > 1) {
				S.sparse_on = true;
				const BlockGeom g1 = block_geom(S, 1);
				k_window_masks<<<dim3((unsigned)((S.rows + 255) / 256), S.nsys), dim3(256), 0, S.sA>>>((const u64 *)S.Wb, S.rows, g1.gb, (const int *)S.died, S.wmask,
				                                                                                      (const SolveState *)S.st, S.ss());
				HIPCHK(hipGetLastError());
			}
		}
		return GF2BV_OK;
	};
	int b = 0;
	if (S.tl_K) {
		const int G = S.impl->G;
		hipStream_t so = S.sC ? S.sC : S.sB;
		bool big_recorded = false;
		for (int p0 = 0; p0 < S.tl_bend; p0 += S.tl_K) {
			const int p1 = p0 + S.tl_K;
			if (p0 > 0) {
				HIPCHK(hipStreamWaitEvent(S.sA, S.evPri, 0));
				if ((rc = enqueue_window_gather(S, p0))) return rc;
			}
			S.tile_hi = (i64)p1 * G / TW;
			for (b = p0; b < p1; b++)
				if ((rc = one_block(b))) return rc;
			S.tile_hi = S.ntiles;
			if ((rc = enqueue_outer_prepare(S, S.sA, p0, p1))) return rc;
			HIPCHK(hipEventRecord(S.evPanelDone, S.sA));
			HIPCHK(hipStreamWaitEvent(so, S.evPanelDone, 0));
			const i64 t_out = S.ntiles;
			const i64 t0 = (i64)p1 * G / TW, t1 = std::min<i64>(t_out, t0 + (i64)S.tl_K * G / TW);
			const bool side = S.kn.outer_side && S.sB != so && S.sB != S.sA;
			if (side) {
				HIPCHK(hipStreamWaitEvent(S.sB, S.evPanelDone, 0));
				if (big_recorded) HIPCHK(hipStreamWaitEvent(S.sB, S.evBig, 0));
				if ((rc = enqueue_outer_apply(S, S.sB, p0, p1, t0, t1))) return rc;
				HIPCHK(hipEventRecord(S.evPri, S.sB));
				if ((rc = enqueue_outer_apply(S, so, p0, p1, t1, t_out))) return rc;
			} else {
				if ((rc = enqueue_outer_apply(S, so, p0, p1, t0, t1))) return rc;
				HIPCHK(hipEventRecord(S.evPri, so));
				if ((rc = enqueue_outer_apply(S, so, p0, p1, t1, t_out))) return rc;
			}
			HIPCHK(hipEventRecord(S.evBig, so));
			big_recorded = true;
		}
		HIPCHK(hipEventRecord(S.evOuter, so));
		b = S.tl_bend;
		HIPCHK(hipStreamWaitEvent(S.sA, S.evPri, 0));
		if (b < S.nblocks && (rc = enqueue_window_gather(S, b))) return rc;
		S.bulk_waits_outer = S.sC != nullptr;
	}
	for (; b < S.nblocks; b++)
		if ((rc = one_block(b))) return rc;
	if ((rc = enqueue_forward_join(S))) return rc;
	tr.mark(S.kn, "forward: all blocks submitted");
	while (optimistic || S.sparse_on) {
		HIPCHK(hipMemcpyAsync(&hst, S.st, sizeof hst, hipMemcpyDeviceToHost, S.sA));
		HIPCHK(hipStreamSynchronize(S.sA));
		if (!hst.poison) break;
		{
			const int pb = hst.poison - 1;
			if ((rc = recover(pb))) return rc;
			optimistic = false;
			if (S.sparse_on && ++S.sparse_giveups > 3) S.sparse_on = false;
			S.sparse_tier = std::min(2, S.sparse_tier + 1);
			general_only = pb;
			for (b = pb; b < S.nblocks; b++)
				if ((rc = one_block(b))) return rc;
			if ((rc = enqueue_forward_join(S))) return rc;
		}
	}
	return enqueue_check_rhs(S);
}

int enqueue_backward(Solver &S, const std::vector<int> &ycols_host)
{
	S.ny = (int)ycols_host.size();
	const i64 nyw = (S.ny + 63) / 64;
	S.ys = round_up(nyw, YTW);
	HIPCHK(pool().alloc((void **)&S.ycols, sizeof(int) * S.ny, S.device));
	HIPCHK(hipMemcpyAsync(S.ycols, ycols_host.data(), sizeof(int) * S.ny, hipMemcpyHostToDevice, S.sA));
	HIPCHK(pool().alloc((void **)&S.Y, sizeof(u64) * std::max<i64>(1, S.maxr) * S.ys, S.device));
	HIPCHK(hipMemsetAsync(S.Y, 0, sizeof(u64) * std::max<i64>(1, S.maxr) * S.ys, S.sA));
	HIPCHK(pool().alloc((void **)&S.out, sizeof(u64) * S.ny * std::max<i64>(1, S.cw), S.device));
	HIPCHK(hipMemsetAsync(S.out, 0, sizeof(u64) * S.ny * std::max<i64>(1, S.cw), S.sA));
	u64 *bmult = S.mult;
	const int rpb = 2048;
	if (S.maxr > 0) {
		const i64 kchunk = std::max<i64>(1, (1ll << 24) / nyw);
		for (i64 k0 = 0; k0 < S.maxr; k0 += kchunk) {
			const i64 waves = std::min(kchunk, S.maxr - k0) * nyw;
			k_extract_y<<<dim3((unsigned)((waves + 3) / 4)), dim3(256), 0, S.sA>>>(S.M, S.srows, S.st, S.urow, S.pivcol,
			                                                                      S.ycols, S.ny, S.Y, S.ys, k0);
		}
		const int ytiles = (int)(S.ys / YTW);
		for (int q = S.npanels - 1; q >= 1; q--) {
			const i64 bound = std::min<i64>((i64)64 * q, S.maxr);
			int g = (int)std::min<i64>(1024, (bound + 255) / 256);
			k_gather_mult_u<<<dim3(g), dim3(256), 0, S.sA>>>(S.M, S.srows, q, S.panels + q, S.urow, bmult);
			const i64 nrb = (bound + rpb - 1) / rpb;
			HIPCHK(launch_ysweep(dim3((unsigned)(ytiles * nrb)), S.sA, S.Y, S.ys, S.maxr, S.panels + q, bmult, ytiles, rpb));
		}
		for (i64 k0 = 0; k0 < S.maxr; k0 += kchunk << 6) {
			const i64 thr = std::min(kchunk << 6, S.maxr - k0) * nyw;
			k_scatter_solution<<<dim3((unsigned)((thr + 255) / 256)), dim3(256), 0, S.sA>>>(S.Y, S.ys, S.st, S.pivcol, S.ny,
			                                                                              S.out, std::max<i64>(1, S.cw), k0);
		}
	}
	HIPCHK(hipGetLastError());
	HIPCHK(hipEventRecord(S.ev2, S.sA));
	return GF2BV_OK;
}

int enqueue_backward_parity(Solver &S, const std::vector<int> &ycols_host)
{
	S.ny = (int)ycols_host.size();
	const i64 cw = std::max<i64>(1, S.cw);
	HIPCHK(pool().alloc((void **)&S.ycols, sizeof(int) * S.ny, S.device));
	HIPCHK(hipMemcpyAsync(S.ycols, ycols_host.data(), sizeof(int) * S.ny, hipMemcpyHostToDevice, S.sA));
	HIPCHK(pool().alloc((void **)&S.out, sizeof(u64) * S.ny * cw, S.device));
	HIPCHK(hipMemsetAsync(S.out, 0, sizeof(u64) * S.ny * cw, S.sA));
	unsigned char *accv = reinterpret_cast<unsigned char *>(S.mult);
	const i64 nacc = std::max<i64>(1, S.maxr);
	HIPCHK(pool().alloc((void **)&S.Y, sizeof(u64) * 64 * 16 * std::max(1, S.npanels), S.device));
	if (S.npanels > 0)
		k_bs_diag<<<dim3(S.npanels), dim3(256), 0, S.sA>>>(S.M, S.srows, S.npanels, S.panels, S.urow, S.Y, SysStride{0, 0}, (i64)0);
	const int ngroups = (S.npanels + GF2_BSG - 1) / GF2_BSG;
	const bool inv = S.kn.bs_inv >= 0 ? S.kn.bs_inv != 0 && ngroups >= 1 : ngroups >= 16;
	if (inv) {
		HIPCHK(pool().alloc((void **)&S.Minv, sizeof(u64) * (size_t)ngroups * 16 * 64 * 16, S.device));
		static std::mutex mu;
		static std::map<int, bool> raised;
		{
			std::lock_guard<std::mutex> lk(mu);
			if (!raised[S.device]) {
				HIPCHK(hipFuncSetAttribute((const void *)k_bs_inv, hipFuncAttributeMaxDynamicSharedMemorySize, GF2_BSINV_LDS));
				raised[S.device] = true;
			}
		}
		k_bs_inv<<<dim3(ngroups), dim3(1024), GF2_BSINV_LDS, S.sA>>>(S.Y, S.npanels, S.panels, S.pivcol, S.Minv);
	}
	for (int v0 = 0; v0 < S.ny; v0 += GF2_BSV) {
		const int nv = std::min(GF2_BSV, S.ny - v0);
		for (int qb = S.npanels; qb > 0; qb -= GF2_BSG) {
			const int qa = std::max(0, qb - GF2_BSG);
			const int waves = (qb - qa) * 64;
			k_bs_far<<<dim3((waves + 3) / 4), dim3(256), 0, S.sA>>>(S.M, S.srows, cw, qa, qb, S.panels, S.urow, S.pivcol, S.ycols + v0, nv,
			                                                        S.out + (i64)v0 * cw, accv, nacc, SysStride{0, 0}, (i64)0);
			if (inv)
				k_bs_near2<<<dim3(1), dim3(1024), 0, S.sA>>>(cw, qa, qb, S.panels, S.pivcol, nv, S.out + (i64)v0 * cw, accv, nacc, S.Minv,
				                                             (S.npanels - qb) / GF2_BSG);
			else
				k_bs_near<<<dim3(1), dim3(256), 0, S.sA>>>(S.Y, cw, qa, qb, S.panels, S.pivcol, nv, S.out + (i64)v0 * cw, accv, nacc,
				                                           SysStride{0, 0}, (i64)0, (i64)0);
		}
	}
	HIPCHK(hipGetLastError());
	HIPCHK(hipEventRecord(S.ev2, S.sA));
	return GF2BV_OK;
}

int enqueue_backward_gang(Solver &S)
{
	S.ny = 1;
	const i64 cw = std::max<i64>(1, S.cw);
	S.h_ycol = (int)S.cols;
	HIPCHK(pool().alloc((void **)&S.ycols, sizeof(int), S.device));
	HIPCHK(hipMemcpyAsync(S.ycols, &S.h_ycol, sizeof(int), hipMemcpyHostToDevice, S.sA));
	HIPCHK(pool().alloc((void **)&S.out, sizeof(u64) * cw * S.nsys, S.device));
	HIPCHK(hipMemsetAsync(S.out, 0, sizeof(u64) * cw * S.nsys, S.sA));
	unsigned char *accv = reinterpret_cast<unsigned char *>(S.mult);
	const i64 nacc = std::max<i64>(1, S.maxr);
	const i64 dgw = (i64)64 * 16 * std::max(1, S.npanels);
	HIPCHK(pool().alloc((void **)&S.Y, sizeof(u64) * dgw * S.nsys, S.device));
	if (S.npanels > 0)
		k_bs_diag<<<dim3(S.npanels, S.nsys), dim3(256), 0, S.sA>>>(S.M, S.srows, S.npanels, S.panels, S.urow, S.Y, S.ss(), dgw);
	for (int qb = S.npanels; qb > 0; qb -= GF2_BSG) {
		const int qa = std::max(0, qb - GF2_BSG);
		const int waves = (qb - qa) * 64;
		k_bs_far<<<dim3((waves + 3) / 4, S.nsys), dim3(256), 0, S.sA>>>(S.M, S.srows, cw, qa, qb, S.panels, S.urow, S.pivcol, S.ycols, 1,
		                                                                S.out, accv, nacc, S.ss(), cw);
		k_bs_near<<<dim3(1, S.nsys), dim3(256), 0, S.sA>>>(S.Y, cw, qa, qb, S.panels, S.pivcol, 1, S.out, accv, nacc, S.ss(), dgw, cw);
	}
	HIPCHK(hipGetLastError());
	HIPCHK(hipEventRecord(S.ev2, S.sA));
	return GF2BV_OK;
}

int enqueue_backsub(Solver &S, const std::vector<int> &ycols)
{
	if ((i64)ycols.size() <= GF2_BS_MAXRHS && !S.kn.ysweep) return enqueue_backward_parity(S, ycols);
	return enqueue_backward(S, ycols);
}

int solver_enqueue(Solver &S)
{
	Trace tr;
	int rc = solver_alloc(S);
	tr.mark(S.kn, "solver_alloc");
	if (rc) return rc;
	rc = enqueue_forward(S);
	tr.mark(S.kn, "enqueue_forward");
	if (rc) return rc;
	if (S.mode == GF2BV_MODE_SINGLE) return enqueue_backsub(S, { (int)S.cols });
	return GF2BV_OK;
}

std::vector<int> m4ri_free_order(const int32_t *piv, i64 rank, i64 cols)
{
	std::vector<int> order(cols);
	for (i64 i = 0; i < cols; i++) order[i] = (int)i;
	for (i64 i = 0; i < rank; i++) std::swap(order[i], order[piv[i]]);
	return std::vector<int>(order.begin() + rank, order.end());
}

int load_free_order(Solver &S)
{
	HIPCHK(hipMemcpyAsync(&S.hst, S.st, sizeof S.hst, hipMemcpyDeviceToHost, S.sA));
	HIPCHK(hipStreamSynchronize(S.sA));
	std::vector<int32_t> piv(S.hst.rank);
	if (S.hst.rank)
		HIPCHK(hipMemcpy(piv.data(), S.pivcol, sizeof(int) * S.hst.rank, hipMemcpyDeviceToHost));
	S.free_order = m4ri_free_order(piv.data(), S.hst.rank, S.cols);
	return GF2BV_OK;
}

int enqueue_export(Solver &S)
{
	HIPCHK(pool().event(&S.evx, true));
	HIPCHK(hipMemcpyAsync(&S.hst, S.st, sizeof S.hst, hipMemcpyDeviceToHost, S.sA));
	S.hout.resize((size_t)S.ny * std::max<i64>(1, S.cw));
	HIPCHK(hipMemcpyAsync(S.hout.data(), S.out, sizeof(u64) * S.hout.size(), hipMemcpyDeviceToHost, S.sA));
	S.hp.resize(std::max(1, S.npanels));
	HIPCHK(hipMemcpyAsync(S.hp.data(), S.panels, sizeof(PanelRec) * S.hp.size(), hipMemcpyDeviceToHost, S.sA));
	S.hpiv.resize(std::max<i64>(1, S.maxr));
	HIPCHK(hipMemcpyAsync(S.hpiv.data(), S.pivcol, sizeof(int) * S.hpiv.size(), hipMemcpyDeviceToHost, S.sA));
	HIPCHK(hipEventRecord(S.evx, S.sA));
	return GF2BV_OK;
}

int finish_begin(Solver &S)
{
	if (S.mode == GF2BV_MODE_AFFINE_SPACE) {
		int rc = load_free_order(S);
		if (rc) return rc;
		std::vector<int> yc;
		if (!S.hst.inconsistent) yc = S.free_order;
		yc.push_back((int)S.cols);
		if ((rc = enqueue_backsub(S, yc))) return rc;
	}
	return enqueue_export(S);
}

int handover_verdict(Solver &S)
{
	if (!S.hst.gate_timeout) return GF2BV_OK;
	if (!S.flag_sync) return fail(GF2BV_ERR_HIP, "a stream hand-over gate timed out on the device");
	forget_concurrency(S.device);
	return GF2BV_RETRY_EVENTS;
}

std::unique_ptr<gf2bv_result> new_result(bool solved, i64 cols, const int32_t *piv, i64 rank, const u64 *origin)
{
	const i64 cw = (cols + 63) / 64;
	std::unique_ptr<gf2bv_result> R(new gf2bv_result());
	R->status = solved ? GF2BV_STATUS_SOLVED : GF2BV_STATUS_INCONSISTENT;
	R->rank = rank;
	R->cw = cw;
	R->dim = cols - rank;
	R->pivots.assign(piv, piv + rank);
	R->origin.assign((size_t)std::max<i64>(1, cw), 0);
	if (solved) std::copy(origin, origin + cw, R->origin.begin());
	return R;
}

std::vector<u64> basis_rows(const u64 *hout, i64 cw, const std::vector<int> &free_order, i64 dim)
{
	const i64 cwx = std::max<i64>(1, cw);
	std::vector<u64> basis((size_t)(dim * cwx), 0);
	for (i64 t = 0; t < dim; t++) {
		u64 *v = basis.data() + (size_t)(t * cwx);
		std::copy(hout + (size_t)(t * cwx), hout + (size_t)(t * cwx + cw), v);
		const int f = free_order[(size_t)t];
		v[f >> 6] |= 1ull << (f & 63);
	}
	return basis;
}

void fill_stats(const Solver &S, gf2bv_result *R);

int finish_end(Solver &S, gf2bv_result **out)
{
	Trace tr;
	HIPCHK(hipStreamSynchronize(S.sA));
	HIPCHK(hipStreamSynchronize(S.sB));
	tr.mark(S.kn, "finish: sync");
	int rc = handover_verdict(S);
	if (rc) return rc;
	const SolveState &hst = S.hst;
	const i64 cwx = std::max<i64>(1, S.cw);
	S.hpiv.resize(hst.rank);
	std::unique_ptr<gf2bv_result> R = new_result(!hst.inconsistent, S.cols, S.hpiv.data(), hst.rank, S.hout.data() + (size_t)((S.ny - 1) * cwx));
	if (!hst.inconsistent && S.mode == GF2BV_MODE_AFFINE_SPACE) R->basis = basis_rows(S.hout.data(), S.cw, S.free_order, R->dim);
	fill_stats(S, R.get());
	tr.mark(S.kn, "finish: result");
	*out = R.release();
	return GF2BV_OK;
}

void fill_stats(const Solver &S, gf2bv_result *R)
{
	const SolveState &hst = S.hst;
	const std::vector<PanelRec> &hp = S.hp;
	const hipEvent_t evx = S.evx;
	gf2bv_stats &st = R->stats;
	st.rows = S.rows; st.cols = S.cols; st.stride_words = S.stride;
	st.rank = R->rank; st.dimension = R->dim; st.status = R->status;
	st.n_panels = S.npanels;
	st.panels_per_sweep = S.impl->G;
	st.tables_per_sweep = S.impl->G * S.impl->T;
	st.table_bits = (64 + S.impl->T - 1) / S.impl->T;
	st.tile_words = TW;
	st.gang_systems = S.view ? S.gang_nsys : S.nsys;
	st.search_handovers = hst.self_giveups;
	st.fast_blocks = hst.fast_blocks;
	{
		const int G = S.impl->G;
		for (int b = 0; b < S.nblocks; b++) {
			const int j0 = b * G, gb = std::min(G, S.npanels - j0), wlo = j0 + gb;
			int pend = 0, any = 0;
			for (int g = 0; g < gb; g++) { any |= hp[j0 + g].p; pend = hp[j0 + g].start + hp[j0 + g].p; }
			if (!any || wlo >= S.wt) continue;
			const double rows_swept = (double)(S.rows - pend);
			st.n_sweeps++;
			st.sweep_words += rows_swept * (double)(S.wt - wlo);
			st.row_xors += rows_swept * (double)(S.impl->T * gb);
			if (S.tl_K && b < S.tl_bend) {
				const int pend_w = (b / S.tl_K + 1) * S.tl_K * G;
				const i64 out_w = S.wt;
				st.outer_blocks++;
				if (pend_w > wlo) { st.hbm_words += rows_swept * (double)(std::min<i64>(pend_w, S.wt) - wlo); st.bulk_launches++; }
				if ((b + 1) % S.tl_K == 0 && out_w > pend_w) { st.hbm_words += rows_swept * (double)(out_w - pend_w); st.bulk_launches += 2; }
			} else { st.hbm_words += rows_swept * (double)(S.wt - wlo); st.bulk_launches++; }
		}
	}
	st.ms_pack = S.ms_pack;
	st.handover_retries = g_attempt;
	(void)hipEventElapsedTime(&st.ms_eliminate, S.ev0, S.ev1);
	(void)hipEventElapsedTime(&st.ms_backsub, S.ev1, S.ev2);
	(void)hipEventElapsedTime(&st.ms_export, S.ev2, evx);
	{
		std::vector<std::pair<float, float>> iv;
		for (size_t i = 0; i + 1 < S.kev.size(); i += 2) {
			float ms = 0, at = 0;
			(void)hipEventElapsedTime(&ms, S.kev[i], S.kev[i + 1]);
			if (hipEventElapsedTime(&at, S.ev0, S.kev[i]) != hipSuccess) { (void)hipGetLastError(); at = iv.empty() ? 0.f : iv.back().second; }
			iv.push_back({ at, at + ms });
		}
		std::sort(iv.begin(), iv.end());
		float lo = 0, hi = -1;
		for (const auto &v : iv) {
			if (hi < 0) { lo = v.first; hi = v.second; }
			else if (v.first <= hi) hi = std::max(hi, v.second);
			else { st.ms_sweep += hi - lo; lo = v.first; hi = v.second; }
		}
		if (hi >= 0) st.ms_sweep += hi - lo;
	}
	st.ms_total = std::chrono::duration<float, std::milli>(std::chrono::steady_clock::now() - S.t_begin).count();
}

int solver_finish(Solver &S, gf2bv_result **out)
{
	int rc = finish_begin(S);
	if (rc) return rc;
	return finish_end(S, out);
}

int make_view(const Solver &S, int s, Solver &V)
{
	V.plan() = S.plan();
	V.view = true;
	V.gang_nsys = S.nsys;
	V.nsys = 1; V.m_stride = 0; V.src_sys_words = 0;
	V.M = S.M + S.m_stride * s;
	V.arena = (char *)S.arena + S.lay.stride * s;
	V.bind(S.lay, V.arena, S.kn.pc);
	V.lay.stride = 0;
	V.sA = S.sA; V.sB = S.sB;
	V.ev0 = S.ev0; V.ev1 = S.ev1; V.ev3 = S.ev3;
	HIPCHK(pool().event(&V.ev2, true));
	return GF2BV_OK;
}

int solve_gang(Solver &S, gf2bv_result **out)
{
	int rc = solver_alloc(S);
	if (rc) return rc;
	rc = enqueue_forward(S);
	if (rc) return rc;
	std::vector<Solver> V(S.nsys);
	for (int s = 0; s < S.nsys; s++) {
		V[s].device = S.device;
		rc = make_view(S, s, V[s]);
		if (rc) return rc;
	}
	if (S.mode == GF2BV_MODE_SINGLE) {
		if (!S.kn.gang_bs)
			for (int s = 0; s < S.nsys; s++) {
				rc = enqueue_backward_parity(V[s], { (int)S.cols });
				if (rc) return rc;
			}
		else {
			rc = enqueue_backward_gang(S);
			if (rc) return rc;
			for (int s = 0; s < S.nsys; s++) {
				V[s].out = S.out + (i64)s * std::max<i64>(1, S.cw); V[s].ny = 1; V[s].own_bs = false;
				HIPCHK(hipEventRecord(V[s].ev2, S.sA));
			}
		}
	}
	for (int s = 0; s < S.nsys; s++) {
		rc = finish_begin(V[s]);
		if (rc) return rc;
	}
	for (int s = 0; s < S.nsys; s++) {
		rc = finish_end(V[s], &out[s]);
		if (rc) return rc;
	}
	if (S.time_kernels) {
		float total = 0;
		for (size_t i = 0; i + 1 < S.kev.size(); i += 2) {
			float ms = 0;
			(void)hipEventElapsedTime(&ms, S.kev[i], S.kev[i + 1]);
			total += ms;
		}
		for (int s = 0; s < S.nsys; s++) out[s]->stats.ms_sweep = total;
	}
	return GF2BV_OK;
}

i64 pick_gang(const Knobs &kn, i64 nsys, i64 rows, i64 cols, i64 free_bytes = -1)
{
	const double per_sys = 1.05 * 8.0 * (double)(rows + 64) * (double)((cols + 64) / 64 + TW + 4 * GF2_GMAX);
	i64 gang = std::max<i64>(2, std::min<i64>(64, (i64)(4.5 * 1073741824.0 / per_sys)));
	gang = std::min(gang, std::max<i64>(1, (nsys + 1) / 2));
	if (gang < nsys) {
		i64 ngangs = (nsys + gang - 1) / gang;
		if (ngangs > 1 && (ngangs & 1)) ngangs++;
		gang = (nsys + ngangs - 1) / ngangs;
	}
	if (gang >= 8) gang = gang / 8 * 8;
// ... 222 lines not shown
			d_src = (const u64 *)d_base; d_stride = wt;
		}
		if (!zero_copy) HIPCHK(hipMemcpyAsync(back.d_in, G.h_in, in_bytes, hipMemcpyHostToDevice, st));
	}
	constexpr int NT = 1024;
	const size_t lds = sizeof(u64) * (size_t)((rows + 512) * small_pitch(wt)) + sizeof(SmallLds);
	{
		static std::mutex mu;
		static std::map<int, bool> raised;
		std::lock_guard<std::mutex> lk(mu);
		if (!raised[device]) {
			HIPCHK(hipFuncSetAttribute((const void *)k_small_solve<NT>, hipFuncAttributeMaxDynamicSharedMemorySize, 160 * 1024 - 256));
			raised[device] = true;
		}
	}
	memset(G.h_out, 0, 16);
	k_small_solve<NT><<<dim3(1), dim3(NT), lds, st>>>(d_src, d_stride, d_dig, d_off, in.bpd, (int)rows, (int)cols, want_basis ? 1 : 0, (unsigned *)G.h_out,
	                                                   kn.small_probe ? (unsigned long long *)(G.h_out + res_bytes) : nullptr);
	HIPCHK(hipGetLastError());
	HIPCHK(hipStreamSynchronize(st));
	const unsigned *ho = (const unsigned *)G.h_out;
	if (kn.small_probe) {
		const unsigned long long *p = (const unsigned long long *)(G.h_out + res_bytes);
		fprintf(stderr, "[gf2bv small %lld x %lld] us: load %.1f candidates %.1f wavefront0 %.1f candidate rows %.1f tables %.1f all rows %.1f read-out %.1f; passes %llu\n",
		        (long long)rows, (long long)cols, p[0] / 100.0, p[1] / 100.0, p[2] / 100.0, p[3] / 100.0, p[4] / 100.0, p[5] / 100.0, p[6] / 100.0, p[7]);
	}
	const i64 rank = ho[0];
	const bool bad = ho[1] != 0;
	if (rank < 0 || rank > cols) return fail(GF2BV_ERR_HIP, "small solve returned an impossible rank");
	const int32_t *pv = (const int32_t *)(G.h_out + 16);
	const u64 *org = (const u64 *)(G.h_out + head);
	std::unique_ptr<gf2bv_result> R = new_result(!bad, cols, pv, rank, org);
	if (!bad && want_basis) {
		const std::vector<int> free_order = m4ri_free_order(pv, rank, cols);
		std::vector<int> slot(cols, -1);
		std::vector<char> isp(cols, 0);
		for (i64 i = 0; i < rank; i++) isp[pv[i]] = 1;
		int j = 0;
		for (i64 c = 0; c < cols; c++) if (!isp[c]) slot[c] = j++;
		const u64 *Y = org + cw;
		R->basis.assign((size_t)R->dim * std::max<i64>(1, cw), 0);
		for (i64 t = 0; t < R->dim; t++) {
			const int f = free_order[(size_t)t];
			u64 *v = R->basis.data() + (size_t)t * cw;
			std::copy(Y + (size_t)slot[f] * cw, Y + (size_t)(slot[f] + 1) * cw, v);
			v[f >> 6] |= 1ull << (f & 63);
		}
	}
	gf2bv_stats &s = R->stats;
	s.rows = rows; s.cols = cols; s.stride_words = wt;
	s.rank = rank; s.dimension = R->dim; s.status = R->status;
	s.n_panels = (int)cw; s.gang_systems = 1; s.tile_words = 0;
	s.small_path = 1;
	s.ms_total = std::chrono::duration<float, std::milli>(std::chrono::steady_clock::now() - t_begin).count();
	*out = R.release();
	return GF2BV_OK;
}

int check_rhs_args(i64 rows, i64 cols, const void *rhs, bool on_device, i64 nrhs, i64 rhs_words)
{
	if (!rhs) return fail(GF2BV_ERR_ARG, "null pointer");
	if (nrhs < 1) return fail(GF2BV_ERR_ARG, "nrhs must be at least 1");
	if (nrhs >= (1ll << 31) - 64 - cols) return fail(GF2BV_ERR_ARG, "too many right-hand sides");
	if (rhs_words < (rows + 63) / 64) return fail(GF2BV_ERR_ARG, "rhs_words does not cover one bit per row");
	if (on_device && ((uintptr_t)rhs & 7)) return fail(GF2BV_ERR_ARG, "the right-hand sides need 8-byte alignment");
	return GF2BV_OK;
}

int pack_coefficients(const MatrixInput &in, i64 rows, i64 cols, i64 ntiles, i64 srows, int device, hipStream_t st, Scratch &scratch, u64 *M)
{
	const i64 cw = (cols + 63) / 64, rw = (rows + 63) / 64;
	if (in.h_off) {
		const i64 ndig = in.h_off[rows];
		uint32_t *d_dig = nullptr;
		i64 *d_off = nullptr;
		HIPCHK(scratch.alloc((void **)&d_dig, sizeof(uint32_t) * std::max<i64>(1, ndig), device));
		HIPCHK(scratch.alloc((void **)&d_off, sizeof(i64) * (rows + 1), device));
		if (ndig) HIPCHK(hipMemcpyAsync(d_dig, in.h_digits, sizeof(uint32_t) * ndig, hipMemcpyHostToDevice, st));
		HIPCHK(hipMemcpyAsync(d_off, in.h_off, sizeof(i64) * (rows + 1), hipMemcpyHostToDevice, st));
		k_pack_digits<<<dim3((unsigned)((ntiles * TW + 255) / 256), (unsigned)std::min<i64>(rows, 65535)), dim3(256), 0, st>>>(
			d_dig, d_off, in.bpd, rows, cols, ntiles * TW, srows, M, SysStride{0, 0}, (i64)0);
	} else {
		const u64 *src = in.d_words;
		i64 sstride = in.stride;
		if (in.h_words) {
			sstride = round_up(cw, 2);
			u64 *tmp = nullptr;
			HIPCHK(scratch.alloc((void **)&tmp, sizeof(u64) * rows * sstride, device));
			HIPCHK(hipMemcpy2DAsync(tmp, sstride * 8, in.h_words, in.stride * 8, cw * 8, rows, hipMemcpyHostToDevice, st));
			src = tmp;
		}
		k_to_tiled<<<dim3((unsigned)rw, (unsigned)((ntiles + 15) / 16)), dim3(256), 0, st>>>(src, sstride, rows, ntiles, cw, srows, M,
		                                                                                      (i64)0, SysStride{0, 0});
	}
	HIPCHK(hipGetLastError());
	return GF2BV_OK;
}

int solve_rhs(const MatrixInput &in, const u64 *rhs, bool rhs_on_device, i64 nrhs, i64 rhs_words, i64 rows, i64 cols, int mode, int device,
              hipStream_t stream, bool time_kernels, gf2bv_result **out)
{
	const i64 cw = (cols + 63) / 64, cwx = std::max<i64>(1, cw), nmw = (nrhs + 63) / 64;
	const i64 wt = (cols + nrhs + 63) / 64, ntiles = tiles_for(wt), srows = slab_rows(rows);
	const i64 rw = (rows + 63) / 64, nrw = ((cols & 63) + nrhs + 63) / 64;
	Solver S;
	S.t_begin = std::chrono::steady_clock::now();
	S.device = device;
	if (in.d_words) S.sA = stream;
	else { HIPCHK(pool().stream(&S.sA, device, false)); S.own_sA = true; }
	S.rows = rows; S.cols = cols; S.mode = mode; S.nrhs = (int)nrhs;
	S.time_kernels = time_kernels;
	S.stride = in.h_off ? ntiles * TW : in.stride;
	if (int rc = alloc_or_nomem((void **)&S.M, sizeof(u64) * ntiles * TW * srows + kOuterSlackBytes, device,
	                            "the matrix widened by the right-hand sides does not fit on the device", "working matrix")) return rc;
	Scratch scratch;
	scratch.sync_first = S.sA;
	HIPCHK(scratch.alloc((void **)&S.rhs_bad, sizeof(u64) * nmw, device));
	hipEvent_t p0, p1;
	HIPCHK(scratch.event(&p0)); HIPCHK(scratch.event(&p1));
	HIPCHK(hipEventRecord(p0, S.sA));
	HIPCHK(hipMemsetAsync(S.rhs_bad, 0, sizeof(u64) * nmw, S.sA));
	int rc;
	if ((rc = pack_coefficients(in, rows, cols, ntiles, srows, S.device, S.sA, scratch, S.M))) return rc;
	const u64 *d_rhs = rhs;
	i64 rhs_stride = rhs_words;
	if (!rhs_on_device) {
		u64 *d = nullptr;
		HIPCHK(scratch.alloc((void **)&d, sizeof(u64) * nrhs * rw, device));
		HIPCHK(hipMemcpy2DAsync(d, rw * 8, rhs, rhs_words * 8, rw * 8, nrhs, hipMemcpyHostToDevice, S.sA));
		d_rhs = d; rhs_stride = rw;
	}
	k_pack_rhs<<<dim3((unsigned)((rw + 3) / 4), (unsigned)std::min<i64>(nrw, 65535)), dim3(256), 0, S.sA>>>(d_rhs, nrhs, rhs_stride, rows, cols,
	                                                                                                  srows, S.M);
	HIPCHK(hipGetLastError());
	HIPCHK(hipEventRecord(p1, S.sA));
	rc = solver_alloc(S);
	if (rc) return rc;
	rc = enqueue_forward(S);
	if (rc) return rc;
	std::vector<u64> bad((size_t)nmw, 0);
	std::vector<int> yc;
	if (mode == GF2BV_MODE_AFFINE_SPACE) {
		if ((rc = load_free_order(S))) return rc;
		HIPCHK(hipMemcpy(bad.data(), S.rhs_bad, sizeof(u64) * nmw, hipMemcpyDeviceToHost));
		bool any_ok = false;
		for (i64 j = 0; j < nrhs && !any_ok; j++) any_ok = !((bad[(size_t)(j >> 6)] >> (j & 63)) & 1);
		if (any_ok) yc = S.free_order;
	}
	const i64 nbasis = (i64)yc.size();
	for (i64 j = 0; j < nrhs; j++) yc.push_back((int)(cols + j));
	if ((rc = enqueue_backsub(S, yc))) return rc;
	HIPCHK(hipMemcpyAsync(bad.data(), S.rhs_bad, sizeof(u64) * nmw, hipMemcpyDeviceToHost, S.sA));
	if ((rc = enqueue_export(S))) return rc;
	HIPCHK(hipStreamSynchronize(S.sA));
	HIPCHK(hipStreamSynchronize(S.sB));
	if ((rc = handover_verdict(S))) return rc;
	(void)hipEventElapsedTime(&S.ms_pack, p0, p1);
	S.hpiv.resize(S.hst.rank);
	const std::vector<u64> basis = basis_rows(S.hout.data(), cw, S.free_order, nbasis);
	std::vector<std::unique_ptr<gf2bv_result>> res((size_t)nrhs);
	for (i64 j = 0; j < nrhs; j++) {
		const bool ok = !((bad[(size_t)(j >> 6)] >> (j & 63)) & 1);
		res[(size_t)j] = new_result(ok, cols, S.hpiv.data(), S.hst.rank, S.hout.data() + (size_t)((nbasis + j) * cwx));
		if (ok && mode == GF2BV_MODE_AFFINE_SPACE) res[(size_t)j]->basis = basis;
		fill_stats(S, res[(size_t)j].get());
	}
	for (i64 j = 0; j < nrhs; j++) out[j] = res[(size_t)j].release();
	return GF2BV_OK;
}


}

struct gf2bv_factor {
	mutable std::mutex mu;
	Solver S;
	i64 rows = 0, cols = 0, tw0 = 0, rw = 0, cw = 0;
	int mode = 0, device = 0;
	i64 rank = 0;
	std::vector<int32_t> piv;
	std::vector<u64> basis;
	gf2bv_stats fst{};
	i64 device_bytes = 0;
	i64 cap_rows = 0;
	std::vector<PanelRec> hp;
	std::vector<int32_t> urow;
	int *died_buf = nullptr;
	bool failed = false;
	~gf2bv_factor()
	{
		if (died_buf) {
			(void)hipSetDevice(device);
			if (S.sA) (void)hipStreamSynchronize(S.sA);
			pool().release(died_buf);
		}
	}
};

namespace {

constexpr i64 kFactorSlots = 64;
const char *kFailedHandle = "the handle is unusable: an append failed after it had started to change it";

void release_backsub(Solver &S)
{
	(void)hipStreamSynchronize(S.sA);
	for (void *p : { (void *)S.Y, (void *)S.ycols, (void *)S.out, (void *)S.Minv }) pool().release(p);
	S.Y = nullptr; S.ycols = nullptr; S.out = nullptr; S.Minv = nullptr;
}

int factor_basis(gf2bv_factor *h, std::vector<u64> &basis)
{
	Solver &S = h->S;
	basis.clear();
	int rc = load_free_order(S);
	if (rc) return rc;
	const i64 dim = h->cols - h->rank;
	if (!dim) return GF2BV_OK;
	if ((rc = enqueue_backsub(S, S.free_order))) return rc;
	std::vector<u64> hout((size_t)(dim * std::max<i64>(1, h->cw)));
	HIPCHK(hipMemcpyAsync(hout.data(), S.out, sizeof(u64) * hout.size(), hipMemcpyDeviceToHost, S.sA));
	HIPCHK(hipStreamSynchronize(S.sA));
	basis = basis_rows(hout.data(), h->cw, S.free_order, dim);
	return GF2BV_OK;
}

i64 factor_device_bytes(const gf2bv_factor *h)
{
	const Solver &S = h->S;
	return (i64)(sizeof(u64) * S.ntiles * TW * S.srows + kOuterSlackBytes + S.lay.stride) + (h->died_buf ? (i64)sizeof(int) * h->cap_rows : 0);
}

int factor_matrix(const MatrixInput &in, i64 rows, i64 cols, int mode, int device, hipStream_t stream, gf2bv_factor **out)
{
	const i64 rw = (rows + 63) / 64, cw = (cols + 63) / 64;
	const i64 tw0 = round_up(cols + kFactorSlots, 128) / 64;
	const i64 wt = tw0 + rw, ntiles = tiles_for(wt), srows = slab_rows(rows);
	std::unique_ptr<gf2bv_factor> h(new gf2bv_factor());
	h->rows = rows; h->cols = cols; h->mode = mode; h->device = device; h->tw0 = tw0; h->rw = rw; h->cw = cw;
	Solver &S = h->S;
	S.t_begin = std::chrono::steady_clock::now();
	S.device = device;
	HIPCHK(pool().stream(&S.sA, device, false));
	S.own_sA = true;
	S.rows = rows; S.cols = cols; S.mode = mode;
	S.nrhs = (int)(wt * 64 - cols);
	S.stride = in.h_off ? ntiles * TW : in.stride;
	if (in.d_words) {
		hipEvent_t e = nullptr;
		HIPCHK(pool().event(&e, false));
		HIPCHK(hipEventRecord(e, stream));
		HIPCHK(hipStreamWaitEvent(S.sA, e, 0));
		pool().release_event(e, false);
	}
	if (int rc = alloc_or_nomem((void **)&S.M, sizeof(u64) * ntiles * TW * srows + kOuterSlackBytes, device,
	                            "the factorization (the matrix and its row transform, about twice the matrix) does not fit on the device", "working matrix")) return rc;
	Scratch scratch;
	scratch.sync_first = S.sA;
	int rc = pack_coefficients(in, rows, cols, ntiles, srows, S.device, S.sA, scratch, S.M);
	if (rc) return rc;
	k_factor_init<<<dim3((unsigned)((rows + 255) / 256), (unsigned)std::min<i64>(wt - (cols >> 6), 64)), dim3(256), 0, S.sA>>>(
		rows, cols, srows, tw0, rw, S.M);
	HIPCHK(hipGetLastError());
	if ((rc = solver_alloc(S))) return rc;
	if ((rc = enqueue_forward(S))) return rc;
	HIPCHK(hipMemcpyAsync(&S.hst, S.st, sizeof S.hst, hipMemcpyDeviceToHost, S.sA));
	S.hp.resize(std::max(1, S.npanels));
	HIPCHK(hipMemcpyAsync(S.hp.data(), S.panels, sizeof(PanelRec) * S.hp.size(), hipMemcpyDeviceToHost, S.sA));
	HIPCHK(hipStreamSynchronize(S.sA));
	HIPCHK(hipStreamSynchronize(S.sB));
	if (S.sC) HIPCHK(hipStreamSynchronize(S.sC));
	if ((rc = handover_verdict(S))) return rc;
	h->rank = S.hst.rank;
	h->piv.resize((size_t)h->rank);
	h->urow.resize((size_t)h->rank);
	if (h->rank) HIPCHK(hipMemcpy(h->piv.data(), S.pivcol, sizeof(int) * h->rank, hipMemcpyDeviceToHost));
	if (h->rank) HIPCHK(hipMemcpy(h->urow.data(), S.urow, sizeof(int) * h->rank, hipMemcpyDeviceToHost));
	h->hp.assign(S.hp.begin(), S.hp.begin() + S.npanels);
	h->cap_rows = rows;
	if (mode == GF2BV_MODE_AFFINE_SPACE && (rc = factor_basis(h.get(), h->basis))) return rc;
	{
		gf2bv_result R;
		R.rank = h->rank; R.dim = cols - h->rank;
		fill_stats(S, &R);
		(void)hipGetLastError();
		h->fst = R.stats;
	}
	release_backsub(S);
	h->device_bytes = factor_device_bytes(h.get());
	*out = h.release();
	return GF2BV_OK;
}

int factor_pass(gf2bv_factor *h, const u64 *d_rhs, i64 np, i64 rhs_stride, hipEvent_t ev[5], std::chrono::steady_clock::time_point t0,
                u64 *acc, u64 *bad, gf2bv_result **out)
{
	Solver &S = h->S;
	const i64 rows = h->rows, cols = h->cols, cw = h->cw, cwx = std::max<i64>(1, cw), rw = h->rw;
	HIPCHK(hipMemsetAsync(acc, 0, sizeof(u64) * std::max<i64>(1, rows), S.sA));
	HIPCHK(hipMemsetAsync(bad, 0, sizeof(u64), S.sA));
	HIPCHK(hipEventRecord(ev[1], S.sA));
	const unsigned gx = (unsigned)((rows + 255) / 256);
	k_apply_transform<<<dim3(gx, (unsigned)((rw + GF2_FT_WORDS - 1) / GF2_FT_WORDS)), dim3(256), 0, S.sA>>>(S.M, rows, S.srows, h->tw0, rw, d_rhs,
	                                                                                                     (int)np, rhs_stride, acc);
	k_put_rhs<<<dim3(gx), dim3(256), 0, S.sA>>>(acc, rows, cols, S.srows, S.M);
	const i64 nrw = ((cols & 63) + np + 63) / 64;
	k_check_rhs_many<<<dim3((unsigned)std::min<i64>(1024, gx), (unsigned)nrw), dim3(256), 0, S.sA>>>(S.M, rows, S.srows, cols, np, S.died, bad);
	HIPCHK(hipGetLastError());
// ... 1043 lines not shown
	(void)hipSetDevice(sp->device);
	if (sp->st) (void)hipStreamSynchronize(sp->st);
	pool().release(sp->d_origin); pool().release(sp->d_basis); pool().release(sp->d_out);
	if (sp->h_out) (void)hipHostFree(sp->h_out);
	if (sp->st) pool().release_stream(sp->st, sp->device, false);
	delete sp;
}

int gf2bv_synth_device(void *d_aug, int64_t rows, int64_t cols, int64_t stride_words, uint64_t seed,
                       int device, void *stream)
{
	if (!d_aug || rows < 0 || cols <= 0 || stride_words < (cols + 1 + 63) / 64 || rows >= (1ll << 20) - 1)
		return fail(GF2BV_ERR_ARG, "bad synthetic shape");
	int rc = check_device(device);
	if (rc) return rc;
	if (rows == 0) return GF2BV_OK;
	hipLaunchKernelGGL(k_synth, dim3((unsigned)((rows + 3) / 4)), dim3(256), 0, (hipStream_t)stream,
	                   (u64 *)d_aug, (i64)rows, (i64)cols, (i64)stride_words, (u64)seed);
	HIPCHK(hipGetLastError());
	return GF2BV_OK;
}

int gf2bv_residual_device(const void *d_aug, int64_t rows, int64_t cols, int64_t stride_words,
                          const uint64_t *x_words, int device, void *stream, int64_t *bad_rows)
{
	if (!d_aug || !x_words || !bad_rows || cols <= 0) return fail(GF2BV_ERR_ARG, "null pointer");
	int rc = check_device(device);
	if (rc) return rc;
	const i64 cw = (cols + 63) / 64;
	u64 *dx = nullptr, *dbad = nullptr;
	HIPCHK(hipMalloc(&dx, sizeof(u64) * cw));
	HIPCHK(hipMalloc(&dbad, sizeof(u64)));
	hipStream_t s = (hipStream_t)stream;
	HIPCHK(hipMemcpyAsync(dx, x_words, sizeof(u64) * cw, hipMemcpyHostToDevice, s));
	HIPCHK(hipMemsetAsync(dbad, 0, sizeof(u64), s));
	if (rows > 0)
		hipLaunchKernelGGL(k_residual, dim3((unsigned)((rows + 3) / 4)), dim3(256), 0, s,
		                   (const u64 *)d_aug, (i64)rows, (i64)cols, (i64)stride_words, dx, dbad);
	u64 h = 0;
	HIPCHK(hipMemcpyAsync(&h, dbad, sizeof h, hipMemcpyDeviceToHost, s));
	HIPCHK(hipStreamSynchronize(s));
	(void)hipFree(dx); (void)hipFree(dbad);
	*bad_rows = (int64_t)h;
	return GF2BV_OK;
}

int gf2bv_kernel_resources(int device, int32_t *out, int n)
{
	return guarded([&]() -> int {
	if (!out || n < 10) return fail(GF2BV_ERR_ARG, "need room for 5 kernels");
	for (int k = 0; k < n; k++) out[k] = 0;
	int rc = check_device(device);
	if (rc) return rc;
	HIPCHK(hipSetDevice(device));
	const void *fn[5] = { (const void *)k_update16<512, false, 3, true, 512>, (const void *)k_block_fast, (const void *)k_narrow_all,
	                      (const void *)k_prio_window, (const void *)k_panel_step };
	for (int k = 0; k < 5; k++) {
		hipFuncAttributes a{};
		HIPCHK(hipFuncGetAttributes(&a, fn[k]));
		out[2 * k] = a.numRegs;
		out[2 * k + 1] = (int32_t)a.sharedSizeBytes;
	}
	if (n >= 13) {
		hipFuncAttributes a{};
		HIPCHK(hipFuncGetAttributes(&a, (const void *)k_update16k_wide));
		out[10] = a.numRegs; out[11] = (int32_t)a.sharedSizeBytes; out[12] = (int32_t)a.localSizeBytes;
	}
	if (n >= 15) {
		hipFuncAttributes a{};
		HIPCHK(hipFuncGetAttributes(&a, (const void *)k_block_fast_narrow));
		out[13] = a.numRegs; out[14] = (int32_t)a.sharedSizeBytes;
	}
	if (n >= 17) {
		hipFuncAttributes a{};
		HIPCHK(hipFuncGetAttributes(&a, (const void *)k_block_sparse<256, 4>));
		out[15] = a.numRegs; out[16] = (int32_t)a.sharedSizeBytes;
	}
	return GF2BV_OK;
	});
}

int gf2bv_stream_ceiling_device(int device, int64_t bytes, double *rmw_gbs, double *read_gbs)
{
	if (!rmw_gbs || !read_gbs || bytes < (1 << 20)) return fail(GF2BV_ERR_ARG, "bad ceiling request");
	int rc = check_device(device);
	if (rc) return rc;
	const int wgs = 2048;
	const i64 per = bytes / 16 / wgs;
	uint4 *buf = nullptr;
	unsigned *sink = nullptr;
	hipError_t e = hipMalloc(&buf, (size_t)per * wgs * 16);
	if (e != hipSuccess) return fail(GF2BV_ERR_NOMEM, "hipMalloc", e);
	HIPCHK(hipMalloc(&sink, 64));
	HIPCHK(hipMemset(buf, 1, (size_t)per * wgs * 16));
	hipEvent_t e0, e1;
	HIPCHK(hipEventCreate(&e0)); HIPCHK(hipEventCreate(&e1));
	const int reps = 5;
	float ms = 0;
	k_rmw_stream<<<dim3(wgs), dim3(1024)>>>(buf, per, 5u);
	HIPCHK(hipEventRecord(e0, nullptr));
	for (int r = 0; r < reps; r++) k_rmw_stream<<<dim3(wgs), dim3(1024)>>>(buf, per, 5u);
	HIPCHK(hipEventRecord(e1, nullptr));
	HIPCHK(hipEventSynchronize(e1));
	HIPCHK(hipEventElapsedTime(&ms, e0, e1));
	*rmw_gbs = 2.0 * (double)per * wgs * 16 * reps / (ms * 1e-3) / 1e9;
	k_read_stream<<<dim3(wgs), dim3(1024)>>>(buf, per, sink);
	HIPCHK(hipEventRecord(e0, nullptr));
	for (int r = 0; r < reps; r++) k_read_stream<<<dim3(wgs), dim3(1024)>>>(buf, per, sink);
	HIPCHK(hipEventRecord(e1, nullptr));
	HIPCHK(hipEventSynchronize(e1));
	HIPCHK(hipEventElapsedTime(&ms, e0, e1));
	*read_gbs = (double)per * wgs * 16 * reps / (ms * 1e-3) / 1e9;
	(void)hipEventDestroy(e0); (void)hipEventDestroy(e1);
	(void)hipFree(buf); (void)hipFree(sink);
	return GF2BV_OK;
}

int gf2bv_lds_clock_device(int device, double *shader_mhz, double *lds_bytes_per_clk_cu)
{
	if (!shader_mhz || !lds_bytes_per_clk_cu) return fail(GF2BV_ERR_ARG, "null pointer");
	int rc = check_device(device);
	if (rc) return rc;
	unsigned long long *d = nullptr, h[3] = { 0, 0, 0 };
	unsigned *sink = nullptr;
	struct Free { unsigned long long *&d; unsigned *&sink; ~Free() { pool().release(d); pool().release(sink); } } guard{ d, sink };
	HIPCHK(pool().alloc((void **)&d, sizeof h, device));
	HIPCHK(pool().alloc((void **)&sink, 64, device));
	int cus = 256;
	(void)hipDeviceGetAttribute(&cus, hipDeviceAttributeMultiprocessorCount, device);
	k_lds_clock<<<dim3(cus), dim3(512)>>>(d, 2000, sink);
	k_lds_clock<<<dim3(cus), dim3(512)>>>(d, 40000, sink);
	HIPCHK(hipGetLastError());
	HIPCHK(hipMemcpy(h, d, sizeof h, hipMemcpyDeviceToHost));
	if (!h[1]) return fail(GF2BV_ERR_HIP, "the clock probe measured nothing");
	*shader_mhz = (double)h[0] / ((double)h[1] / 100.0);
	*lds_bytes_per_clk_cu = (double)h[2] * 1024.0 / (double)h[0];
	return GF2BV_OK;
}

int gf2bv_device_alloc(int device, int64_t bytes, void **d_ptr)
{
	if (!d_ptr || bytes < 0) return fail(GF2BV_ERR_ARG, "bad alloc request");
	int rc = check_device(device);
	if (rc) return rc;
	hipError_t e = pool().malloc_retry(d_ptr, (size_t)std::max<i64>(bytes, 16), device);
	if (e != hipSuccess) return fail(GF2BV_ERR_NOMEM, "hipMalloc", e);
	return GF2BV_OK;
}
namespace {
struct HostPool {
	std::mutex mu;
	struct Buf { void *p; size_t bytes; };
	std::vector<Buf> idle;
	std::unordered_map<void *, size_t> live;
};
HostPool *host_pool_ptr() { static HostPool *p = new HostPool(); return p; }
}
int gf2bv_host_alloc(int64_t bytes, void **h_ptr)
{
	if (!h_ptr || bytes < 0) return fail(GF2BV_ERR_ARG, "bad alloc request");
	*h_ptr = nullptr;
	const size_t need = std::max<size_t>((size_t)bytes, 64);
	HostPool &P = *host_pool_ptr();
	{
		std::lock_guard<std::mutex> lk(P.mu);
		for (size_t i = 0; i < P.idle.size(); i++)
			if (P.idle[i].bytes >= need && P.idle[i].bytes <= 2 * need + ((size_t)1 << 20)) {
				*h_ptr = P.idle[i].p; P.live[*h_ptr] = P.idle[i].bytes;
				P.idle.erase(P.idle.begin() + i);
				return GF2BV_OK;
			}
	}
	int n = 0;
	if (hipGetDeviceCount(&n) != hipSuccess || n <= 0) return fail(GF2BV_ERR_NODEVICE, "no HIP device visible");
	void *p = nullptr;
	const size_t cap = need + need / 8;
	hipError_t e = hipHostMalloc(&p, cap, hipHostMallocDefault);
	if (e != hipSuccess) { (void)hipGetLastError(); return fail(GF2BV_ERR_NOMEM, "hipHostMalloc", e); }
	std::lock_guard<std::mutex> lk(P.mu);
	P.live[p] = cap;
	*h_ptr = p;
	return GF2BV_OK;
}
void gf2bv_host_free(void *h_ptr)
{
	if (!h_ptr) return;
	HostPool &P = *host_pool_ptr();
	void *drop = nullptr;
	{
		std::lock_guard<std::mutex> lk(P.mu);
		auto it = P.live.find(h_ptr);
		if (it == P.live.end()) return;
		const size_t bytes = it->second;
		P.live.erase(it);
		size_t kept = 0;
		for (const auto &b : P.idle) kept += b.bytes;
		const size_t cap_mb = (size_t)Knobs::read(Knobs::kHostPool).host_pool_mb;
		if (P.idle.size() < 4 && kept + bytes <= (cap_mb << 20)) P.idle.push_back({ h_ptr, bytes });
		else drop = h_ptr;
	}
	if (drop) (void)hipHostFree(drop);
}

int64_t gf2bv_host_pool_trim(void)
{
	HostPool &P = *host_pool_ptr();
	std::vector<HostPool::Buf> drop;
	{
		std::lock_guard<std::mutex> lk(P.mu);
		drop.swap(P.idle);
	}
	int64_t bytes = 0;
	for (const auto &b : drop) { bytes += (int64_t)b.bytes; (void)hipHostFree(b.p); }
	return bytes;
}

int64_t gf2bv_plan_gang(int64_t nsys, int64_t rows, int64_t cols, int64_t free_bytes)
{
	if (nsys <= 0 || rows <= 0 || cols <= 0 || free_bytes < 0) return 0;
	return pick_gang(Knobs::read(), nsys, rows, cols, free_bytes);
}

int gf2bv_knob_dump(char *buf, int64_t n)
{
	return catching([&]() -> int {
	const std::string s = Knobs::read().dump();
	if (!buf || (int64_t)s.size() >= n) return fail(GF2BV_ERR_ARG, "null pointer, or a buffer too small for the knob dump");
	memcpy(buf, s.c_str(), s.size() + 1);
	return GF2BV_OK;
	});
}

int64_t gf2bv_pool_trim(int device)
{
	if (check_device(device)) return -1;
	return (int64_t)pool().trim(device);
}
int64_t gf2bv_pool_idle_bytes(int device)
{
	if (device < 0) return -1;
	Pool &P = pool();
	std::lock_guard<std::mutex> lk(P.mu);
	size_t bytes = 0;
	auto bf = P.big_free.find(device);
	if (bf != P.big_free.end()) for (const Pool::Big &b : bf->second) bytes += b.bytes;
	for (auto &kv : P.free_bufs) if (kv.first.first == device) bytes += kv.first.second * kv.second.size();
	return (int64_t)bytes;
}
int gf2bv_device_free(int device, void *d_ptr)
{
	int rc = check_device(device);
	if (rc) return rc;
	HIPCHK(hipFree(d_ptr));
	return GF2BV_OK;
}
int gf2bv_device_upload(int device, void *d_dst, const void *h_src, int64_t bytes)
{
	int rc = check_device(device);
	if (rc) return rc;
	HIPCHK(hipMemcpy(d_dst, h_src, (size_t)bytes, hipMemcpyHostToDevice));
	return GF2BV_OK;
}
int gf2bv_device_download(int device, void *h_dst, const void *d_src, int64_t bytes)
{
	int rc = check_device(device);
	if (rc) return rc;
	HIPCHK(hipMemcpy(h_dst, d_src, (size_t)bytes, hipMemcpyDeviceToHost));
	return GF2BV_OK;
}

#ifdef GF2_SPARSE_DEBUG
extern "C" int gf2bv_sparse_probe_read(unsigned long long *w, int reset)
{
	HIPCHK(hipDeviceSynchronize());
	HIPCHK(hipMemcpyFromSymbol(w, HIP_SYMBOL(gf2_sparse_probe), sizeof(gf2_sparse_probe)));
	if (reset) { unsigned long long z[8] = { 0 }; HIPCHK(hipMemcpyToSymbol(HIP_SYMBOL(gf2_sparse_probe), z, sizeof z)); }
	return GF2BV_OK;
}
#endif
#ifdef GF2_STEP_PROBE
int gf2bv_probe_set(int j0)
{
	HIPCHK(hipMemcpyToSymbol(HIP_SYMBOL(gf2_probe_j0), &j0, sizeof(int)));
	void *p = nullptr;
	HIPCHK(hipGetSymbolAddress(&p, HIP_SYMBOL(gf2_probe_upd))); HIPCHK(hipMemset(p, 0, sizeof(gf2_probe_upd)));
	HIPCHK(hipGetSymbolAddress(&p, HIP_SYMBOL(gf2_probe_wg))); HIPCHK(hipMemset(p, 0, sizeof(gf2_probe_wg)));
	HIPCHK(hipGetSymbolAddress(&p, HIP_SYMBOL(gf2_probe_un))); HIPCHK(hipMemset(p, 0, sizeof(gf2_probe_un)));
	return GF2BV_OK;
}
int gf2bv_probe_read_update(unsigned long long *upd)
{
	HIPCHK(hipDeviceSynchronize());
	HIPCHK(hipMemcpyFromSymbol(upd, HIP_SYMBOL(gf2_probe_upd), sizeof(gf2_probe_upd)));
	return GF2BV_OK;
}
int gf2bv_probe_read_gj(unsigned long long *w)
{
	HIPCHK(hipDeviceSynchronize());
	HIPCHK(hipMemcpyFromSymbol(w, HIP_SYMBOL(gf2_probe_gj), sizeof(gf2_probe_gj)));
	return GF2BV_OK;
}
int gf2bv_probe_read_fast(unsigned long long *w)
{
	HIPCHK(hipDeviceSynchronize());
	HIPCHK(hipMemcpyFromSymbol(w, HIP_SYMBOL(gf2_probe_fast), sizeof(gf2_probe_fast)));
	return GF2BV_OK;
}
int gf2bv_probe_read_wave(unsigned long long *w)
{
	HIPCHK(hipDeviceSynchronize());
	HIPCHK(hipMemcpyFromSymbol(w, HIP_SYMBOL(gf2_probe_wave), sizeof(gf2_probe_wave)));
	return GF2BV_OK;
}
int gf2bv_probe_read(unsigned long long *wg, unsigned long long *un)
{
	HIPCHK(hipDeviceSynchronize());
	HIPCHK(hipMemcpyFromSymbol(wg, HIP_SYMBOL(gf2_probe_wg), sizeof(gf2_probe_wg)));
	HIPCHK(hipMemcpyFromSymbol(un, HIP_SYMBOL(gf2_probe_un), sizeof(gf2_probe_un)));
	return GF2BV_OK;
}
#endif

}

namespace {

constexpr i64 kQuadMaxRank = 256;
constexpr i64 kQuadMaxPoints = 1ll << 22;
constexpr i64 kQuadMaxCand = 1ll << 22;
constexpr int kQuadMaxEnum = 40;
constexpr int kQuadMaxDepth = 8;

inline bool qbit(const u64 *v, i64 i) { return (v[i >> 6] >> (i & 63)) & 1; }
inline void qflip(u64 *v, i64 i) { v[i >> 6] ^= 1ull << (i & 63); }
inline void qxor(u64 *d, const u64 *s, i64 n) { for (i64 k = 0; k < n; k++) d[k] ^= s[k]; }
inline bool qzero(const u64 *v, i64 n) { for (i64 k = 0; k < n; k++) if (v[k]) return false; return true; }
inline void qxor_above(u64 *d, const u64 *s, i64 e, i64 W)
{
	const i64 w0 = (e + 1) >> 6;
	if (w0 >= W) return;
	d[w0] ^= s[w0] & (~0ull << ((e + 1) & 63));
	for (i64 w = w0 + 1; w < W; w++) d[w] ^= s[w];
}

struct QuadTimes { double reduce = 0, forms = 0, affine = 0, search = 0, relin = 0, total = 0; i64 levels = 0, candidates = 0; };
thread_local QuadTimes g_quad_times;

inline double ms_since(std::chrono::steady_clock::time_point t0)
{
	return std::chrono::duration<double, std::milli>(std::chrono::steady_clock::now() - t0).count();
}

struct QuadPlan {
	i64 n = 0, S = 0, N = 0, words = 0, d = 0, dw = 1, r = 0, W = 1;
	std::vector<u64> origin, V, T;
	std::vector<i64> kpiv;
	i64 m0 = 0;
	std::vector<u64> lin, qaff;
	std::vector<int> pair_i, pair_j, sup_idx;
	std::vector<i64> sup_off;
	std::vector<u64> M;
	bool inconsistent = false;
	std::vector<int> sub_var;
// ... 2186 lines not shown
```

Before: 8.083 billion.

## Defer poison check, fuse back-substitution link kernel, and pack export into one copy

In single-solution mode the optimistic forward pass no longer blocks the host to read the poison flag. The tail runs ahead, and the solve resumes from the poisoned block only if the exported state shows poison. Back-substitution gets a block-per-row far kernel and a fused link kernel that combines the near solve with a precomputed adjacency. Right-hand-side columns are passed by value instead of being uploaded. Export packs state, output, panels and pivots into one device buffer and does a single pinned copy, and the host pool gains a small-buffer list. This adds a short spin-wait, a speculative path that may have to be redone, and considerably more complexity.

```diff
diff --git a/gf2bv_amd/csrc/gf2_kernels.hip.h b/gf2bv_amd/csrc/gf2_kernels.hip.h
--- a/gf2bv_amd/csrc/gf2_kernels.hip.h
+++ b/gf2bv_amd/csrc/gf2_kernels.hip.h
@@ -2712,6 +2712,7 @@
 	M += blockIdx.y * ss.m_words;
 	died = sys_at(died, blockIdx.y * ss.arena_bytes);
 	st = sys_at(st, blockIdx.y * ss.arena_bytes);
+	if (st->poison) return;
 	int bad = 0;
 	for (i64 i = (i64)blockIdx.x * blockDim.x + threadIdx.x; i < rows; i += (i64)gridDim.x * blockDim.x)
 		if (died[i] == GF2_NEVER) bad |= (int)((M[tidx(i, cols >> 6, srows)] >> (cols & 63)) & 1);
@@ -3049,9 +3050,50 @@
 #define GF2_BSV 8
 #define GF2_BS_MAXRHS 64
 
+struct BsCols { int c[GF2_BSV]; };
+
+__device__ __forceinline__ unsigned
+bs_far_row(const u64 *__restrict__ M, i64 srows, i64 cw, i64 row, int pw, i64 wbeg, const BsCols &yc, int ny,
+           const u64 *__restrict__ X, unsigned *sh)
+{
+	const int t = threadIdx.x & 255, lane = t & 63, wave = t >> 6;
+	int y = 0;
+	if (t < ny) {
+		const int c = yc.c[t];
+		if ((c >> 6) >= pw) y = (int)((M[tidx(row, c >> 6, srows)] >> (c & 63)) & 1);
+	}
+	u64 par[GF2_BSV];
+#pragma unroll
+	for (int v = 0; v < GF2_BSV; v++) par[v] = 0;
+	for (i64 base = wbeg + t; base < cw; base += 1024) {
+		u64 m[4];
+		i64 wc[4];
+#pragma unroll
+		for (int j = 0; j < 4; j++) {
+			const i64 w = base + 256 * j;
+			wc[j] = w < cw ? w : cw - 1;
+			m[j] = M[tidx(row, wc[j], srows)];
+			if (w >= cw) m[j] = 0;
+		}
+#pragma unroll
+		for (int j = 0; j < 4; j++)
+#pragma unroll
+			for (int v = 0; v < GF2_BSV; v++)
+				if (v < ny) par[v] ^= m[j] & X[(i64)v * cw + wc[j]];
+	}
+	unsigned bits = 0;
+#pragma unroll
+	for (int v = 0; v < GF2_BSV; v++)
+		if (v < ny) bits |= (unsigned)(__popcll(__ballot(__popcll(par[v]) & 1)) & 1) << v;
+	const unsigned yb = (unsigned)__ballot(y);
+	if (lane == 0) sh[wave] = wave == 0 ? bits ^ yb : bits;
+	__syncthreads();
+	return sh[0] ^ sh[1] ^ sh[2] ^ sh[3];
+}
+
 __global__ void __launch_bounds__(256)
 k_bs_far(const u64 *__restrict__ M, i64 srows, i64 cw, int qa, int qb, const PanelRec *__restrict__ panels,
-         const int *__restrict__ urow, const int *__restrict__ pivcol, const int *__restrict__ ycols, int ny,
+         const int *__restrict__ urow, const int *__restrict__ pivcol, BsCols yc, int ny,
          const u64 *__restrict__ X, unsigned char *__restrict__ accv, i64 nacc, SysStride ss, i64 x_sys_words)
 {
 	{
@@ -3059,32 +3101,14 @@
 		M += blockIdx.y * ss.m_words; X += blockIdx.y * x_sys_words;
 		panels = sys_at(panels, ao); urow = sys_at(urow, ao); pivcol = sys_at(pivcol, ao); accv = sys_at(accv, ao);
 	}
-	const int lane = threadIdx.x & 63;
-	const i64 wv = ((i64)blockIdx.x * blockDim.x + threadIdx.x) >> 6;
+	__shared__ unsigned sh[4];
 	const int kbeg = panels[qa].start;
 	const int kend = panels[qb - 1].start + panels[qb - 1].p;
-	const i64 k = kbeg + wv;
+	const i64 k = kbeg + (i64)blockIdx.x;
 	if (k >= kend) return;
-	const i64 row = urow[k];
-	u64 par[GF2_BSV];
-#pragma unroll
-	for (int v = 0; v < GF2_BSV; v++) par[v] = 0;
-	for (i64 w = qb + lane; w < cw; w += 64) {
-		const u64 m = M[tidx(row, w, srows)];
-#pragma unroll
-		for (int v = 0; v < GF2_BSV; v++)
-			if (v < ny) par[v] ^= m & X[(i64)v * cw + w];
-	}
-	const int pw = pivcol[k] >> 6;
-#pragma unroll
-	for (int v = 0; v < GF2_BSV; v++) {
-		if (v >= ny) break;
-		int bit = __popcll(par[v]) & 1;
-		bit = __popcll(__ballot(bit)) & 1;
-		const int c = ycols[v];
-		const int y = ((c >> 6) >= pw) ? (int)((M[tidx(row, c >> 6, srows)] >> (c & 63)) & 1) : 0;
-		if (lane == 0) accv[(i64)v * nacc + k] = (unsigned char)(bit ^ y);
-	}
+	const unsigned bits = bs_far_row(M, srows, cw, urow[k], pivcol[k] >> 6, qb, yc, ny, X, sh);
+	if (threadIdx.x == 0)
+		for (int v = 0; v < ny; v++) accv[(i64)v * nacc + k] = (unsigned char)((bits >> v) & 1);
 }
 
 #define GF2_BSINV_LDS (16 * 64 * 16 * 8 + 256 * 8 * 8 + 1024 + 64)
@@ -3145,38 +3169,112 @@
 	for (int e = t; e < 16 * 64 * 16; e += 1024) dst[e] = R[e];
 }
 
+#define GF2_BSC 8
 __global__ void __launch_bounds__(1024)
-k_bs_near2(i64 cw, int qa, int qb, const PanelRec *__restrict__ panels, const int *__restrict__ pivcol, int ny,
-           u64 *__restrict__ X, const unsigned char *__restrict__ accv, i64 nacc, const u64 *__restrict__ Minv, int gidx)
-{
+k_bs_link(const u64 *__restrict__ M, i64 srows, i64 cw, int qa, int qb, int hqa, int hqb, i64 hbeg, BsCols yc, int ny,
+          u64 *__restrict__ X, u64 *__restrict__ pre, i64 npre, const u64 *__restrict__ Adj, const int *__restrict__ srow,
+          const u64 *__restrict__ Minv, int gidx)
+{
+	static_assert(GF2_TW == 2, "16-byte tiles");
+	static_assert(GF2_BSV * GF2_BSC == 64, "workgroup 0: one lane per (right-hand side, share)");
 	__shared__ u64 aL[GF2_BSG];
-	const int lane = threadIdx.x & 63, i = threadIdx.x >> 6, nb = qb - qa;
-	const bool onp = i < nb;
-	const uint4 *rowp = reinterpret_cast<const uint4 *>(Minv + (i64)gidx * (16 * 64 * 16) + ((i64)(onp ? i : 0) * 64 + lane) * 16);
-	uint4 q[8];
-#pragma unroll
-	for (int z = 0; z < 8; z++) q[z] = rowp[z];
-	const PanelRec rec = panels[qa + (onp ? i : 0)];
-	const int kk = rec.start + lane;
-	const bool piv = onp && lane < rec.p;
-	const int pcb = piv ? (pivcol[kk] & 63) : 0;
-	for (int v = 0; v < ny; v++) {
-		const u64 word = wave_or(piv ? (u64)(accv[(i64)v * nacc + kk] & 1) << pcb : 0ull);
-		if (lane == 0) aL[i] = word;
-		__syncthreads();
-		u64 acc = 0;
-#pragma unroll
-		for (int z = 0; z < 8; z++)
-			acc ^= ((((u64)q[z].y << 32) | q[z].x) & aL[2 * z]) ^ ((((u64)q[z].w << 32) | q[z].z) & aL[2 * z + 1]);
-		const u64 xw = __ballot(__popcll(acc) & 1);
-		if (lane == 0 && onp) X[(i64)v * cw + qa + i] = xw;
-		__syncthreads();
+	__shared__ u64 Xs[GF2_BSV][GF2_BSG];
+	__shared__ u64 wsh[GF2_BSV][16];
+	const int t = threadIdx.x;
+	if (blockIdx.x == 0) {
+		const int lane = t & 63, i = t >> 6, nb = qb - qa;
+		if (nb <= 0) return;
+		const bool onp = i < nb;
+		const i64 slot = (i64)(qa + (onp ? i : 0)) * 64 + lane;
+		const uint4 *rowp = reinterpret_cast<const uint4 *>(Minv + (i64)gidx * (16 * 64 * 16) + ((i64)(onp ? i : 0) * 64 + lane) * 16);
+		const uint4 *adjp = reinterpret_cast<const uint4 *>(Adj + slot * 16);
+		uint4 q[8], a[8];
+#pragma unroll
+		for (int z = 0; z < 8; z++) q[z] = rowp[z];
+#pragma unroll
+		for (int z = 0; z < 8; z++) a[z] = adjp[z];
+		const bool piv = onp && srow[slot] >= 0;
+		u64 pw = ((lane >> 3) < ny && onp) ? pre[(i64)lane * npre + qa + i] : 0ull;
+#pragma unroll
+		for (int m = 1; m < GF2_BSC; m <<= 1)
+			pw ^= ((u64)(unsigned)__shfl_xor((int)(unsigned)(pw >> 32), m) << 32) | (unsigned)__shfl_xor((int)(unsigned)pw, m);
+		if (t < GF2_BSV * GF2_BSG) {
+			const int v = t >> 4, j = t & 15;
+			Xs[v][j] = (v < ny && qb + j < cw) ? X[(i64)v * cw + qb + j] : 0ull;
+		}
+		__syncthreads();
+		for (int v = 0; v < ny; v++) {
+			u64 acc = 0;
+#pragma unroll
+			for (int z = 0; z < 8; z++)
+				acc ^= ((((u64)a[z].y << 32) | a[z].x) & Xs[v][2 * z]) ^ ((((u64)a[z].w << 32) | a[z].z) & Xs[v][2 * z + 1]);
+			const u64 word = __ballot(piv && ((__popcll(acc) ^ (int)(readlane64(pw, GF2_BSC * v) >> lane)) & 1));
+			if (lane == 0) aL[i] = word;
+			__syncthreads();
+			acc = 0;
+#pragma unroll
+			for (int z = 0; z < 8; z++)
+				acc ^= ((((u64)q[z].y << 32) | q[z].x) & aL[2 * z]) ^ ((((u64)q[z].w << 32) | q[z].z) & aL[2 * z + 1]);
+			const u64 xw = __ballot(__popcll(acc) & 1);
+			if (lane == 0 && onp) X[(i64)v * cw + qa + i] = xw;
+			__syncthreads();
+		}
+		return;
+	}
+	const int lane = t & 63, wave = t >> 6;
+	const int panel = hqa + (int)(blockIdx.x - 1) / GF2_BSC, share = (int)(blockIdx.x - 1) % GF2_BSC;
+	const int sr = srow[(i64)panel * 64 + lane];
+	const bool valid = sr >= 0;
+	const i64 row = valid ? sr : 0;
+	int y = 0;
+	if (share == 0 && wave < ny) {
+		const int c = yc.c[wave];
+		if ((c >> 6) >= panel) y = (int)((M[tidx(row, c >> 6, srows)] >> (c & 63)) & 1);
+	}
+	u64 par[GF2_BSV];
+#pragma unroll
+	for (int v = 0; v < GF2_BSV; v++) par[v] = 0;
+	const i64 t1 = (cw + 1) >> 1;
+	for (i64 base = (hbeg >> 1) + share * 16 + wave; base < t1; base += 4 * 16 * GF2_BSC) {
+		uint4 m[4];
+		i64 tc[4];
+#pragma unroll
+		for (int j = 0; j < 4; j++) {
+			const i64 tl = base + j * 16 * GF2_BSC;
+			tc[j] = tl < t1 ? tl : t1 - 1;
+			m[j] = *reinterpret_cast<const uint4 *>(M + tidx(row, 2 * tc[j], srows));
+			if (tl >= t1) m[j] = make_uint4(0, 0, 0, 0);
+		}
+#pragma unroll
+		for (int j = 0; j < 4; j++) {
+			const i64 w0 = 2 * tc[j], w1 = w0 + 1;
+			const u64 lo = w0 >= hbeg ? (((u64)m[j].y << 32) | m[j].x) : 0ull, hi = w1 < cw ? (((u64)m[j].w << 32) | m[j].z) : 0ull;
+			const i64 x0 = w0 >= hbeg ? w0 : w1, x1 = w1 < cw ? w1 : w0;
+#pragma unroll
+			for (int v = 0; v < GF2_BSV; v++)
+				if (v < ny) par[v] ^= (lo & X[(i64)v * cw + x0]) ^ (hi & X[(i64)v * cw + x1]);
+		}
+	}
+	const u64 yb = __ballot(valid && y);
+#pragma unroll
+	for (int v = 0; v < GF2_BSV; v++)
+		if (v < ny) {
+			const u64 w = __ballot(valid && (__popcll(par[v]) & 1));
+			if (lane == 0) wsh[v][wave] = v == wave ? w ^ yb : w;
+		}
+	__syncthreads();
+	if (t < ny) {
+		u64 w = 0;
+#pragma unroll
+		for (int z = 0; z < 16; z++) w ^= wsh[t][z];
+		pre[((i64)t * GF2_BSC + share) * npre + panel] = w;
 	}
 }
 
 __global__ void __launch_bounds__(256)
 k_bs_diag(const u64 *__restrict__ M, i64 srows, int npanels, const PanelRec *__restrict__ panels,
-          const int *__restrict__ urow, u64 *__restrict__ Dg, SysStride ss, i64 dg_sys_words)
+          const int *__restrict__ urow, u64 *__restrict__ Dg, SysStride ss, i64 dg_sys_words,
+          const int *__restrict__ pivcol, i64 cw, u64 *__restrict__ Adj, int *__restrict__ srow)
 {
 	{
 		const i64 ao = blockIdx.y * ss.arena_bytes;
@@ -3199,6 +3297,20 @@
 	uint4 *dst = reinterpret_cast<uint4 *>(Dg + ((i64)q * 64 + r) * 16 + 4 * q4);
 	dst[0] = make_uint4((unsigned)v[0], (unsigned)(v[0] >> 32), (unsigned)v[1], (unsigned)(v[1] >> 32));
 	dst[1] = make_uint4((unsigned)v[2], (unsigned)(v[2] >> 32), (unsigned)v[3], (unsigned)(v[3] >> 32));
+	if (Adj && on) {
+		const i64 slot = (i64)q * 64 + (pivcol[rec.start + r] & 63);
+		const int gq = npanels - (npanels - 1 - q) / GF2_BSG * GF2_BSG;
+#pragma unroll
+		for (int m = 0; m < 4; m++) {
+			const i64 w = gq + 4 * q4 + m;
+			v[m] = M[tidx(ur, w < cw ? w : cw - 1, srows)];
+			if (w >= cw) v[m] = 0;
+		}
+		uint4 *ad = reinterpret_cast<uint4 *>(Adj + slot * 16 + 4 * q4);
+		ad[0] = make_uint4((unsigned)v[0], (unsigned)(v[0] >> 32), (unsigned)v[1], (unsigned)(v[1] >> 32));
+		ad[1] = make_uint4((unsigned)v[2], (unsigned)(v[2] >> 32), (unsigned)v[3], (unsigned)(v[3] >> 32));
+		if (q4 == 0) srow[slot] = ur;
+	}
 }
 
 __global__ void __launch_bounds__(256)
@@ -3257,6 +3369,22 @@
 		}
 		if (t < nb) X[(i64)v * cw + qa + t] = Xn[t];
 		__syncthreads();
+	}
+}
+
+__global__ void __launch_bounds__(256)
+k_export_pack(const unsigned *__restrict__ st, i64 n_st, const unsigned *__restrict__ out, i64 n_out,
+              const unsigned *__restrict__ panels, i64 n_pan, const unsigned *__restrict__ pivcol, i64 n_piv, unsigned *__restrict__ dst)
+{
+	const i64 n = n_st + n_out + n_pan + n_piv;
+	for (i64 e = (i64)blockIdx.x * blockDim.x + threadIdx.x; e < n; e += (i64)gridDim.x * blockDim.x) {
+		i64 r = e;
+		unsigned v;
+		if (r < n_st) v = st[r];
+		else if ((r -= n_st) < n_out) v = out[r];
+		else if ((r -= n_out) < n_pan) v = panels[r];
+		else v = pivcol[r - n_pan];
+		dst[e] = v;
 	}
 }
 
diff --git a/gf2bv_amd/csrc/gf2_solver.hip b/gf2bv_amd/csrc/gf2_solver.hip
--- a/gf2bv_amd/csrc/gf2_solver.hip
+++ b/gf2bv_amd/csrc/gf2_solver.hip
@@ -546,6 +546,9 @@
 	bool optimistic = true;
 	bool xcd_pin = true;
 	int sync_base = 0;
+	bool defer_tail = false;
+	bool tail_deferred = false;
+	bool bs_reuse = false;
 	int units = 0;
 	bool sparse_on = false;
 	int sparse_giveups = 0;
@@ -553,12 +556,13 @@
 	int narrow_rpt = 1;
 	i64 ys = 0;
 	int ny = 0;
-	int h_ycol = 0;
 	i64 maxr = 0;
 	int npanels = 0, nblocks = 0;
 	i64 wt = 0, cw = 0;
 
 	std::vector<int> free_order;
+	std::vector<unsigned> xstage;
+	i64 xn[4] = { 0, 0, 0, 0 };
 	SolveState hst{};
 	std::vector<u64> hout;
 	std::vector<PanelRec> hp;
@@ -634,6 +638,9 @@
 	hipEvent_t ev0 = nullptr, ev1 = nullptr, ev2 = nullptr, ev3 = nullptr;
 	std::vector<hipEvent_t> evA, evPrio, kev, waitPrio;
 	hipEvent_t evx = nullptr;
+	unsigned *xdev = nullptr;
+	void *xhost = nullptr;
+	i64 xcap = 0;
 };
 
 struct Solver : SolverPlan, ArenaPtrs, SolverHandles {
@@ -645,12 +652,13 @@
 	~Solver() { release(); }
 	void release()
 	{
-		if (!arena && !M && !tmp_src && !Y && !ycols && !out && !sA && !sB && !ev0) return;
+		if (!arena && !M && !tmp_src && !Y && !ycols && !out && !sA && !sB && !ev0 && !xdev && !xhost) return;
 		(void)hipSetDevice(device);
 		Pool &P = pool();
 		if (view) {
-			if (sA && (Y || ycols || out)) (void)hipStreamSynchronize(sA);
+			if (sA && (Y || ycols || out || xdev)) (void)hipStreamSynchronize(sA);
 			if (own_bs) for (void *p : { (void *)Y, (void *)ycols, (void *)out, (void *)Minv }) P.release(p);
+			P.release(xdev);
 			P.release_event(ev2, true);
 			P.release_event(evx, true);
 			arena = nullptr; M = nullptr; sA = sB = nullptr; ev0 = ev1 = ev3 = nullptr;
@@ -658,7 +666,8 @@
 			if (sC) (void)hipStreamSynchronize(sC);
 			if (sB) (void)hipStreamSynchronize(sB);
 			if (arena || M) (void)hipStreamSynchronize(sA);
-			for (void *p : { arena, (void *)Y, (void *)ycols, (void *)out, (void *)Minv, (void *)(ext_M ? nullptr : M), (void *)tmp_src }) P.release(p);
+			for (void *p : { arena, (void *)Y, (void *)ycols, (void *)out, (void *)Minv, (void *)(ext_M ? nullptr : M), (void *)tmp_src, (void *)xdev }) P.release(p);
+			gf2bv_host_free(xhost);
 			for (hipEvent_t e : { ev0, ev1, ev2, ev3, evx }) P.release_event(e, true);
 			for (hipEvent_t e : { evOuter, evPri, evPanelDone, evBig }) P.release_event(e, false);
 			if (sC) P.release_stream(sC, device, nsys > 1 ? 3 : 1);
@@ -1158,10 +1167,10 @@
 	return GF2BV_OK;
 }
 
-int enqueue_forward(Solver &S)
+int enqueue_forward(Solver &S, int resume_from = -1)
 {
 	Trace tr;
-	int rc = enqueue_forward_begin(S, true);
+	int rc = resume_from < 0 ? enqueue_forward_begin(S, true) : GF2BV_OK;
 	if (rc) return rc;
 	bool optimistic = false;
 	SolveState hst{};
@@ -1215,6 +1224,21 @@
 		}
 		return GF2BV_OK;
 	};
+	auto resume = [&](int pb) -> int {
+		int r;
+		if ((r = recover(pb))) return r;
+		optimistic = false;
+		if (S.sparse_on && ++S.sparse_giveups > 3) S.sparse_on = false;
+		S.sparse_tier = std::min(2, S.sparse_tier + 1);
+		general_only = pb;
+		for (int blk = pb; blk < S.nblocks; blk++)
+			if ((r = one_block(blk))) return r;
+		return enqueue_forward_join(S);
+	};
+	if (resume_from >= 0) {
+		if ((rc = resume(resume_from))) return rc;
+		return enqueue_check_rhs(S);
+	}
 	int b = 0;
 	if (S.tl_K) {
 		const int G = S.impl->G;
@@ -1260,23 +1284,20 @@
 		if ((rc = one_block(b))) return rc;
 	if ((rc = enqueue_forward_join(S))) return rc;
 	tr.mark(S.kn, "forward: all blocks submitted");
-	while (optimistic || S.sparse_on) {
+	S.tail_deferred = S.defer_tail && optimistic && !S.sparse_on;
+	while (!S.tail_deferred && (optimistic || S.sparse_on)) {
 		HIPCHK(hipMemcpyAsync(&hst, S.st, sizeof hst, hipMemcpyDeviceToHost, S.sA));
 		HIPCHK(hipStreamSynchronize(S.sA));
 		if (!hst.poison) break;
-		{
-			const int pb = hst.poison - 1;
-			if ((rc = recover(pb))) return rc;
-			optimistic = false;
-			if (S.sparse_on && ++S.sparse_giveups > 3) S.sparse_on = false;
-			S.sparse_tier = std::min(2, S.sparse_tier + 1);
-			general_only = pb;
-			for (b = pb; b < S.nblocks; b++)
-				if ((rc = one_block(b))) return rc;
-			if ((rc = enqueue_forward_join(S))) return rc;
-		}
+		if ((rc = resume(hst.poison - 1))) return rc;
 	}
 	return enqueue_check_rhs(S);
+}
+
+hipError_t bs_buffer(Solver &S, void **p, size_t bytes)
+{
+	if (S.bs_reuse && *p) return hipSuccess;
+	return pool().alloc(p, bytes, S.device);
 }
 
 int enqueue_backward(Solver &S, const std::vector<int> &ycols_host)
@@ -1284,11 +1305,11 @@
 	S.ny = (int)ycols_host.size();
 	const i64 nyw = (S.ny + 63) / 64;
 	S.ys = round_up(nyw, YTW);
-	HIPCHK(pool().alloc((void **)&S.ycols, sizeof(int) * S.ny, S.device));
+	HIPCHK(bs_buffer(S, (void **)&S.ycols, sizeof(int) * S.ny));
 	HIPCHK(hipMemcpyAsync(S.ycols, ycols_host.data(), sizeof(int) * S.ny, hipMemcpyHostToDevice, S.sA));
-	HIPCHK(pool().alloc((void **)&S.Y, sizeof(u64) * std::max<i64>(1, S.maxr) * S.ys, S.device));
+	HIPCHK(bs_buffer(S, (void **)&S.Y, sizeof(u64) * std::max<i64>(1, S.maxr) * S.ys));
 	HIPCHK(hipMemsetAsync(S.Y, 0, sizeof(u64) * std::max<i64>(1, S.maxr) * S.ys, S.sA));
-	HIPCHK(pool().alloc((void **)&S.out, sizeof(u64) * S.ny * std::max<i64>(1, S.cw), S.device));
+	HIPCHK(bs_buffer(S, (void **)&S.out, sizeof(u64) * S.ny * std::max<i64>(1, S.cw)));
 	HIPCHK(hipMemsetAsync(S.out, 0, sizeof(u64) * S.ny * std::max<i64>(1, S.cw), S.sA));
 	u64 *bmult = S.mult;
 	const int rpb = 2048;
@@ -1322,19 +1343,29 @@
 {
 	S.ny = (int)ycols_host.size();
 	const i64 cw = std::max<i64>(1, S.cw);
-	HIPCHK(pool().alloc((void **)&S.ycols, sizeof(int) * S.ny, S.device));
-	HIPCHK(hipMemcpyAsync(S.ycols, ycols_host.data(), sizeof(int) * S.ny, hipMemcpyHostToDevice, S.sA));
-	HIPCHK(pool().alloc((void **)&S.out, sizeof(u64) * S.ny * cw, S.device));
+	HIPCHK(bs_buffer(S, (void **)&S.out, sizeof(u64) * S.ny * cw));
 	HIPCHK(hipMemsetAsync(S.out, 0, sizeof(u64) * S.ny * cw, S.sA));
 	unsigned char *accv = reinterpret_cast<unsigned char *>(S.mult);
 	const i64 nacc = std::max<i64>(1, S.maxr);
-	HIPCHK(pool().alloc((void **)&S.Y, sizeof(u64) * 64 * 16 * std::max(1, S.npanels), S.device));
-	if (S.npanels > 0)
-		k_bs_diag<<<dim3(S.npanels), dim3(256), 0, S.sA>>>(S.M, S.srows, S.npanels, S.panels, S.urow, S.Y, SysStride{0, 0}, (i64)0);
 	const int ngroups = (S.npanels + GF2_BSG - 1) / GF2_BSG;
 	const bool inv = S.kn.bs_inv >= 0 ? S.kn.bs_inv != 0 && ngroups >= 1 : ngroups >= 16;
+	const size_t nslots = (size_t)ngroups * GF2_BSG * 64, minv_words = nslots * 16;
+	u64 *Adj = nullptr;
+	int *srow = nullptr;
+	u64 *pre = nullptr;
+	const i64 npre = (i64)ngroups * GF2_BSG;
 	if (inv) {
-		HIPCHK(pool().alloc((void **)&S.Minv, sizeof(u64) * (size_t)ngroups * 16 * 64 * 16, S.device));
+		HIPCHK(bs_buffer(S, (void **)&S.Minv, sizeof(u64) * minv_words * 2 + sizeof(int) * nslots + sizeof(u64) * GF2_BSV * GF2_BSC * (size_t)npre));
+		Adj = S.Minv + minv_words;
+		srow = reinterpret_cast<int *>(Adj + minv_words);
+		pre = reinterpret_cast<u64 *>(srow + nslots);
+		HIPCHK(hipMemsetAsync(srow, 0xff, sizeof(int) * nslots, S.sA));
+	}
+	HIPCHK(bs_buffer(S, (void **)&S.Y, sizeof(u64) * 64 * 16 * std::max(1, S.npanels)));
+	if (S.npanels > 0)
+		k_bs_diag<<<dim3(S.npanels), dim3(256), 0, S.sA>>>(S.M, S.srows, S.npanels, S.panels, S.urow, S.Y, SysStride{0, 0}, (i64)0,
+		                                                   S.pivcol, cw, Adj, srow);
+	if (inv) {
 		static std::mutex mu;
 		static std::map<int, bool> raised;
 		{
@@ -1348,17 +1379,26 @@
 	}
 	for (int v0 = 0; v0 < S.ny; v0 += GF2_BSV) {
 		const int nv = std::min(GF2_BSV, S.ny - v0);
+		BsCols yc{};
+		for (int v = 0; v < nv; v++) yc.c[v] = ycols_host[(size_t)(v0 + v)];
+		u64 *X = S.out + (i64)v0 * cw;
+		if (inv) {
+			const int q0 = std::max(0, S.npanels - GF2_BSG);
+			k_bs_link<<<dim3(1 + GF2_BSC * (S.npanels - q0)), dim3(1024), 0, S.sA>>>(S.M, S.srows, cw, 0, 0, q0, S.npanels, (i64)S.npanels + GF2_BSG, yc, nv,
+			                                                                   X, pre, npre, Adj, srow, S.Minv, 0);
+			for (int qb = S.npanels; qb > 0; qb -= GF2_BSG) {
+				const int qa = std::max(0, qb - GF2_BSG), hqa = std::max(0, qa - GF2_BSG);
+				k_bs_link<<<dim3(1 + GF2_BSC * (qa - hqa)), dim3(1024), 0, S.sA>>>(S.M, S.srows, cw, qa, qb, hqa, qa, (i64)qb, yc, nv,
+				                                                             X, pre, npre, Adj, srow, S.Minv, (S.npanels - qb) / GF2_BSG);
+			}
+			continue;
+		}
 		for (int qb = S.npanels; qb > 0; qb -= GF2_BSG) {
 			const int qa = std::max(0, qb - GF2_BSG);
-			const int waves = (qb - qa) * 64;
-			k_bs_far<<<dim3((waves + 3) / 4), dim3(256), 0, S.sA>>>(S.M, S.srows, cw, qa, qb, S.panels, S.urow, S.pivcol, S.ycols + v0, nv,
-			                                                        S.out + (i64)v0 * cw, accv, nacc, SysStride{0, 0}, (i64)0);
-			if (inv)
-				k_bs_near2<<<dim3(1), dim3(1024), 0, S.sA>>>(cw, qa, qb, S.panels, S.pivcol, nv, S.out + (i64)v0 * cw, accv, nacc, S.Minv,
-				                                             (S.npanels - qb) / GF2_BSG);
-			else
-				k_bs_near<<<dim3(1), dim3(256), 0, S.sA>>>(S.Y, cw, qa, qb, S.panels, S.pivcol, nv, S.out + (i64)v0 * cw, accv, nacc,
-				                                           SysStride{0, 0}, (i64)0, (i64)0);
+			k_bs_far<<<dim3((qb - qa) * 64), dim3(256), 0, S.sA>>>(S.M, S.srows, cw, qa, qb, S.panels, S.urow, S.pivcol, yc, nv,
+			                                                       X, accv, nacc, SysStride{0, 0}, (i64)0);
+			k_bs_near<<<dim3(1), dim3(256), 0, S.sA>>>(S.Y, cw, qa, qb, S.panels, S.pivcol, nv, X, accv, nacc,
+			                                           SysStride{0, 0}, (i64)0, (i64)0);
 		}
 	}
 	HIPCHK(hipGetLastError());
@@ -1370,9 +1410,8 @@
 {
 	S.ny = 1;
 	const i64 cw = std::max<i64>(1, S.cw);
-	S.h_ycol = (int)S.cols;
-	HIPCHK(pool().alloc((void **)&S.ycols, sizeof(int), S.device));
-	HIPCHK(hipMemcpyAsync(S.ycols, &S.h_ycol, sizeof(int), hipMemcpyHostToDevice, S.sA));
+	BsCols yc{};
+	yc.c[0] = (int)S.cols;
 	HIPCHK(pool().alloc((void **)&S.out, sizeof(u64) * cw * S.nsys, S.device));
 	HIPCHK(hipMemsetAsync(S.out, 0, sizeof(u64) * cw * S.nsys, S.sA));
 	unsigned char *accv = reinterpret_cast<unsigned char *>(S.mult);
@@ -1380,12 +1419,12 @@
 	const i64 dgw = (i64)64 * 16 * std::max(1, S.npanels);
 	HIPCHK(pool().alloc((void **)&S.Y, sizeof(u64) * dgw * S.nsys, S.device));
 	if (S.npanels > 0)
-		k_bs_diag<<<dim3(S.npanels, S.nsys), dim3(256), 0, S.sA>>>(S.M, S.srows, S.npanels, S.panels, S.urow, S.Y, S.ss(), dgw);
+		k_bs_diag<<<dim3(S.npanels, S.nsys), dim3(256), 0, S.sA>>>(S.M, S.srows, S.npanels, S.panels, S.urow, S.Y, S.ss(), dgw,
+		                                                           (const int *)nullptr, cw, (u64 *)nullptr, (int *)nullptr);
 	for (int qb = S.npanels; qb > 0; qb -= GF2_BSG) {
 		const int qa = std::max(0, qb - GF2_BSG);
-		const int waves = (qb - qa) * 64;
-		k_bs_far<<<dim3((waves + 3) / 4, S.nsys), dim3(256), 0, S.sA>>>(S.M, S.srows, cw, qa, qb, S.panels, S.urow, S.pivcol, S.ycols, 1,
-		                                                                S.out, accv, nacc, S.ss(), cw);
+		k_bs_far<<<dim3((qb - qa) * 64, S.nsys), dim3(256), 0, S.sA>>>(S.M, S.srows, cw, qa, qb, S.panels, S.urow, S.pivcol, yc, 1,
+		                                                               S.out, accv, nacc, S.ss(), cw);
 		k_bs_near<<<dim3(1, S.nsys), dim3(256), 0, S.sA>>>(S.Y, cw, qa, qb, S.panels, S.pivcol, 1, S.out, accv, nacc, S.ss(), dgw, cw);
 	}
 	HIPCHK(hipGetLastError());
@@ -1405,6 +1444,7 @@
 	int rc = solver_alloc(S);
 	tr.mark(S.kn, "solver_alloc");
 	if (rc) return rc;
+	S.defer_tail = S.mode == GF2BV_MODE_SINGLE;
 	rc = enqueue_forward(S);
 	tr.mark(S.kn, "enqueue_forward");
 	if (rc) return rc;
@@ -1433,15 +1473,45 @@
 
 int enqueue_export(Solver &S)
 {
-	HIPCHK(pool().event(&S.evx, true));
-	HIPCHK(hipMemcpyAsync(&S.hst, S.st, sizeof S.hst, hipMemcpyDeviceToHost, S.sA));
-	S.hout.resize((size_t)S.ny * std::max<i64>(1, S.cw));
-	HIPCHK(hipMemcpyAsync(S.hout.data(), S.out, sizeof(u64) * S.hout.size(), hipMemcpyDeviceToHost, S.sA));
-	S.hp.resize(std::max(1, S.npanels));
-	HIPCHK(hipMemcpyAsync(S.hp.data(), S.panels, sizeof(PanelRec) * S.hp.size(), hipMemcpyDeviceToHost, S.sA));
-	S.hpiv.resize(std::max<i64>(1, S.maxr));
-	HIPCHK(hipMemcpyAsync(S.hpiv.data(), S.pivcol, sizeof(int) * S.hpiv.size(), hipMemcpyDeviceToHost, S.sA));
+	if (!S.evx) HIPCHK(pool().event(&S.evx, true));
+	S.xn[0] = (i64)(sizeof(SolveState) / 4);
+	S.xn[1] = S.out ? 2 * (i64)S.ny * std::max<i64>(1, S.cw) : 0;
+	S.xn[2] = (i64)(sizeof(PanelRec) / 4) * std::max(1, S.npanels);
+	S.xn[3] = std::max<i64>(1, S.maxr);
+	const i64 n = S.xn[0] + S.xn[1] + S.xn[2] + S.xn[3];
+	if (n > S.xcap) {
+		pool().release(S.xdev); S.xdev = nullptr;
+		gf2bv_host_free(S.xhost); S.xhost = nullptr;
+		S.xcap = 0;
+		HIPCHK(pool().alloc((void **)&S.xdev, sizeof(unsigned) * n, S.device));
+		if (!S.view) { int rc = gf2bv_host_alloc((int64_t)(sizeof(unsigned) * n), &S.xhost); if (rc) return rc; }
+		S.xcap = n;
+	}
+	if (S.view) S.xstage.resize((size_t)n);
+	void *dst = S.view ? (void *)S.xstage.data() : S.xhost;
+	k_export_pack<<<dim3((unsigned)std::min<i64>(1024, (n + 255) / 256)), dim3(256), 0, S.sA>>>(
+		(const unsigned *)S.st, S.xn[0], (const unsigned *)S.out, S.xn[1], (const unsigned *)S.panels, S.xn[2], (const unsigned *)S.pivcol, S.xn[3], S.xdev);
+	HIPCHK(hipGetLastError());
+	HIPCHK(hipMemcpyAsync(dst, S.xdev, sizeof(unsigned) * n, hipMemcpyDeviceToHost, S.sA));
 	HIPCHK(hipEventRecord(S.evx, S.sA));
+	return GF2BV_OK;
+}
+
+int export_wait(Solver &S)
+{
+	HIPCHK(hipStreamSynchronize(S.sA));
+	HIPCHK(hipStreamSynchronize(S.sB));
+	const unsigned *src = S.view ? S.xstage.data() : (const unsigned *)S.xhost;
+	memcpy(&S.hst, src, sizeof S.hst);
+	src += S.xn[0];
+	S.hout.resize((size_t)(S.xn[1] / 2));
+	memcpy(S.hout.data(), src, sizeof(unsigned) * S.xn[1]);
+	src += S.xn[1];
+	S.hp.resize((size_t)std::max(1, S.npanels));
+	memcpy(S.hp.data(), src, sizeof(unsigned) * S.xn[2]);
+	src += S.xn[2];
+	S.hpiv.resize((size_t)S.xn[3]);
+	memcpy(S.hpiv.data(), src, sizeof(unsigned) * S.xn[3]);
 	return GF2BV_OK;
 }
 
@@ -1498,11 +1568,24 @@
 int finish_end(Solver &S, gf2bv_result **out)
 {
 	Trace tr;
-	HIPCHK(hipStreamSynchronize(S.sA));
-	HIPCHK(hipStreamSynchronize(S.sB));
+	if (S.tail_deferred) {
+		(void)hipEventSynchronize(S.ev1);
+		const auto t0 = std::chrono::steady_clock::now();
+		while (hipEventQuery(S.evx) == hipErrorNotReady && std::chrono::steady_clock::now() - t0 < std::chrono::milliseconds(3)) {}
+		(void)hipGetLastError();
+	}
+	int rc = export_wait(S);
+	if (rc) return rc;
+	if (S.tail_deferred && S.hst.poison) {
+		S.tail_deferred = false;
+		if ((rc = enqueue_forward(S, S.hst.poison - 1))) return rc;
+		S.bs_reuse = true;
+		if ((rc = enqueue_backsub(S, { (int)S.cols }))) return rc;
+		if ((rc = enqueue_export(S))) return rc;
+		if ((rc = export_wait(S))) return rc;
+	}
 	tr.mark(S.kn, "finish: sync");
-	int rc = handover_verdict(S);
-	if (rc) return rc;
+	if ((rc = handover_verdict(S))) return rc;
 	const SolveState &hst = S.hst;
 	const i64 cwx = std::max<i64>(1, S.cw);
 	S.hpiv.resize(hst.rank);
@@ -2031,8 +2114,7 @@
 	if ((rc = enqueue_backsub(S, yc))) return rc;
 	HIPCHK(hipMemcpyAsync(bad.data(), S.rhs_bad, sizeof(u64) * nmw, hipMemcpyDeviceToHost, S.sA));
 	if ((rc = enqueue_export(S))) return rc;
-	HIPCHK(hipStreamSynchronize(S.sA));
-	HIPCHK(hipStreamSynchronize(S.sB));
+	if ((rc = export_wait(S))) return rc;
 	if ((rc = handover_verdict(S))) return rc;
 	(void)hipEventElapsedTime(&S.ms_pack, p0, p1);
 	S.hpiv.resize(S.hst.rank);
@@ -3382,6 +3464,9 @@
 	std::mutex mu;
 	struct Buf { void *p; size_t bytes; };
 	std::vector<Buf> idle;
+	static constexpr size_t kSmall = (size_t)4 << 20;
+	std::vector<Buf> idle_small;
+	std::vector<Buf> &idle_for(size_t bytes) { return bytes <= kSmall ? idle_small : idle; }
 	std::unordered_map<void *, size_t> live;
 };
 HostPool *host_pool_ptr() { static HostPool *p = new HostPool(); return p; }
@@ -3394,12 +3479,13 @@
 	HostPool &P = *host_pool_ptr();
 	{
 		std::lock_guard<std::mutex> lk(P.mu);
-		for (size_t i = 0; i < P.idle.size(); i++)
-			if (P.idle[i].bytes >= need && P.idle[i].bytes <= 2 * need + ((size_t)1 << 20)) {
-				*h_ptr = P.idle[i].p; P.live[*h_ptr] = P.idle[i].bytes;
-				P.idle.erase(P.idle.begin() + i);
-				return GF2BV_OK;
-			}
+		for (std::vector<HostPool::Buf> *list : { &P.idle_small, &P.idle })
+			for (size_t i = 0; i < list->size(); i++)
+				if ((*list)[i].bytes >= need && (*list)[i].bytes <= 2 * need + ((size_t)1 << 20)) {
+					*h_ptr = (*list)[i].p; P.live[*h_ptr] = (*list)[i].bytes;
+					list->erase(list->begin() + i);
+					return GF2BV_OK;
+				}
 	}
 	int n = 0;
 	if (hipGetDeviceCount(&n) != hipSuccess || n <= 0) return fail(GF2BV_ERR_NODEVICE, "no HIP device visible");
@@ -3426,7 +3512,8 @@
 		size_t kept = 0;
 		for (const auto &b : P.idle) kept += b.bytes;
 		const size_t cap_mb = (size_t)Knobs::read(Knobs::kHostPool).host_pool_mb;
-		if (P.idle.size() < 4 && kept + bytes <= (cap_mb << 20)) P.idle.push_back({ h_ptr, bytes });
+		std::vector<HostPool::Buf> &list = P.idle_for(bytes);
+		if (list.size() < 4 && kept + bytes <= (cap_mb << 20)) list.push_back({ h_ptr, bytes });
 		else drop = h_ptr;
 	}
 	if (drop) (void)hipHostFree(drop);
@@ -3439,6 +3526,8 @@
 	{
 		std::lock_guard<std::mutex> lk(P.mu);
 		drop.swap(P.idle);
+		drop.insert(drop.end(), P.idle_small.begin(), P.idle_small.end());
+		P.idle_small.clear();
 	}
 	int64_t bytes = 0;
 	for (const auto &b : drop) { bytes += (int64_t)b.bytes; (void)hipHostFree(b.p); }
```

Result: faster. 8.187 billion, median of 6 (+1.3%).
